# YujiaoShi/HighlyAccurate

Hardware: AMD Instinct MI355X
Metric: image-pairs/sec through N-iter LM pose loop, KITTI shapes (higher is better)
Workload: dtype bf16; 1 GPU; BASELINE configs[1]: LM_S2GP.forward(mode='test'), sat 512x512, grd 256x1024, VGG-16 two-branch, level 3, 5 LM iters x 3 levels, 3-DoF, random-init weights; pairs_per_gpu=32, global_batch=32, parallelism=batch-sharded x1, no collective

## Files before the change

highlyaccurate_amd/csrc/conv_kernels.h:

```cpp
#pragma once
#include "common.h"
#include <type_traits>

typedef __bf16 bf16;
typedef _Float16 f16;
using f32x16 = __attribute__((ext_vector_type(16))) float;
using bf16x8 = __attribute__((ext_vector_type(8))) __bf16;
using f16x8 = __attribute__((ext_vector_type(8))) _Float16;
using f16x4 = __attribute__((ext_vector_type(4))) _Float16;

struct split32 {
  float v;
  split32() = default;
  __host__ __device__ explicit split32(float f) : v(f) {}
  __host__ __device__ explicit operator float() const { return v; }
};
template <typename T> struct Prec { static constexpr bool SPLIT = false; static constexpr int CEPL = 16 / (int)sizeof(T); };
template <> struct Prec<split32> { static constexpr bool SPLIT = true; static constexpr int CEPL = 8; };

__device__ __host__ __forceinline__ float split_scale(unsigned amax_bits) {
  int E = (int)(amax_bits >> 23) & 0xff;
  E = E < 81 ? 81 : (E > 201 ? 201 : E);
  const unsigned bits = (unsigned)(127 + 141 - E) << 23;
  float f;
  __builtin_memcpy(&f, &bits, 4);
  return f;
}
__device__ __forceinline__ void split4(float x0, float x1, float x2, float x3, float s, uint2& hi, uint2& lo) {
  unsigned h01, h23, l01, l23;
  asm("v_fma_mixlo_f16 %0, %4, %8, 0\n\t"
      "v_fma_mixlo_f16 %1, %6, %8, 0\n\t"
      "v_fma_mixhi_f16 %0, %5, %8, 0\n\t"
      "v_fma_mixhi_f16 %1, %7, %8, 0\n\t"
      "v_fma_mixlo_f16 %2, %4, %8, -%0 op_sel_hi:[0,0,1]\n\t"
      "v_fma_mixlo_f16 %3, %6, %8, -%1 op_sel_hi:[0,0,1]\n\t"
      "v_fma_mixhi_f16 %2, %5, %8, -%0 op_sel:[0,0,1] op_sel_hi:[0,0,1]\n\t"
      "v_fma_mixhi_f16 %3, %7, %8, -%1 op_sel:[0,0,1] op_sel_hi:[0,0,1]"
      : "=&v"(h01), "=&v"(h23), "=&v"(l01), "=&v"(l23) : "v"(x0), "v"(x1), "v"(x2), "v"(x3), "v"(s));
  hi = make_uint2(h01, h23);
  lo = make_uint2(l01, l23);
}

#ifndef HLA_TU_DTYPE
#define HLA_TU_DTYPE -1
#endif
#if HLA_TU_DTYPE == 0
typedef float TuT;
#elif HLA_TU_DTYPE == 1
typedef bf16 TuT;
#elif HLA_TU_DTYPE == 2
typedef f16 TuT;
#elif HLA_TU_DTYPE == 3
typedef split32 TuT;
#endif

template <typename T> __device__ __forceinline__ void mma16(f32x16& acc, const uint4& w, const uint4& p);
template <> __device__ __forceinline__ void mma16<bf16>(f32x16& acc, const uint4& w, const uint4& p) {
  acc = __builtin_amdgcn_mfma_f32_32x32x16_bf16(__builtin_bit_cast(bf16x8, w), __builtin_bit_cast(bf16x8, p), acc, 0, 0, 0);
}
template <> __device__ __forceinline__ void mma16<f16>(f32x16& acc, const uint4& w, const uint4& p) {
  acc = __builtin_amdgcn_mfma_f32_32x32x16_f16(__builtin_bit_cast(f16x8, w), __builtin_bit_cast(f16x8, p), acc, 0, 0, 0);
}
template <> __device__ __forceinline__ void mma16<split32>(f32x16& acc, const uint4& w, const uint4& p) {
  acc = __builtin_amdgcn_mfma_f32_32x32x16_f16(__builtin_bit_cast(f16x8, w), __builtin_bit_cast(f16x8, p), acc, 0, 0, 0);
}
template <> __device__ __forceinline__ void mma16<float>(f32x16& acc, const uint4& w, const uint4& p) {
  acc = __builtin_amdgcn_mfma_f32_32x32x2f32(__uint_as_float(w.x), __uint_as_float(p.x), acc, 0, 0, 0);
  acc = __builtin_amdgcn_mfma_f32_32x32x2f32(__uint_as_float(w.y), __uint_as_float(p.y), acc, 0, 0, 0);
  acc = __builtin_amdgcn_mfma_f32_32x32x2f32(__uint_as_float(w.z), __uint_as_float(p.z), acc, 0, 0, 0);
  acc = __builtin_amdgcn_mfma_f32_32x32x2f32(__uint_as_float(w.w), __uint_as_float(p.w), acc, 0, 0, 0);
}

typedef short v4s __attribute__((ext_vector_type(4)));

template <typename T> struct KStep;
template <> struct KStep<bf16> { static constexpr int PX = 16; };
template <> struct KStep<f16> { static constexpr int PX = 16; };
template <> struct KStep<float> { static constexpr int PX = 8; };

template <typename T> __device__ __forceinline__ uint4 frag_kmajor(const char* tile, int stride, int px0, int ch0, int lane);
template <> __device__ __forceinline__ uint4 frag_kmajor<bf16>(const char* tile, int stride, int px0, int ch0, int lane) {
  const int t = lane & 15, i0 = ch0 + 16 * ((lane >> 4) & 1), k0 = px0 + 8 * (lane >> 5);
  const char* p = tile + (k0 + (t >> 2)) * stride + (i0 + 4 * (t & 3)) * 2;
  const v4s lo = __builtin_amdgcn_ds_read_tr16_b64_v4i16((__attribute__((address_space(3))) v4s*)(p));
  const v4s hi = __builtin_amdgcn_ds_read_tr16_b64_v4i16((__attribute__((address_space(3))) v4s*)(p + 4 * stride));
  uint4 r;
  __builtin_memcpy(&r.x, &lo, 8);
  __builtin_memcpy(&r.z, &hi, 8);
  return r;
}
template <> __device__ __forceinline__ uint4 frag_kmajor<f16>(const char* tile, int stride, int px0, int ch0, int lane) {
  return frag_kmajor<bf16>(tile, stride, px0, ch0, lane);
}
template <> __device__ __forceinline__ uint4 frag_kmajor<float>(const char* tile, int stride, int px0, int ch0, int lane) {
  const char* p = tile + (px0 + (lane >> 5)) * stride + (ch0 + (lane & 31)) * 4;
  uint4 r;
  r.x = *(const unsigned*)(p); r.y = *(const unsigned*)(p + 2 * stride);
  r.z = *(const unsigned*)(p + 4 * stride); r.w = *(const unsigned*)(p + 6 * stride);
  return r;
}
template <typename T> __device__ __forceinline__ uint4 frag_ones();
template <> __device__ __forceinline__ uint4 frag_ones<bf16>() { return make_uint4(0x3F803F80u, 0x3F803F80u, 0x3F803F80u, 0x3F803F80u); }
template <> __device__ __forceinline__ uint4 frag_ones<f16>() { return make_uint4(0x3C003C00u, 0x3C003C00u, 0x3C003C00u, 0x3C003C00u); }
template <> __device__ __forceinline__ uint4 frag_ones<float>() { return make_uint4(0x3F800000u, 0x3F800000u, 0x3F800000u, 0x3F800000u); }

__device__ __forceinline__ void store4(bf16* p, float a, float b, float c, float d) {
  const bf16 h[4] = {(bf16)a, (bf16)b, (bf16)c, (bf16)d};
  *(uint2*)p = __builtin_bit_cast(uint2, h);
}
__device__ __forceinline__ void store4(f16* p, float a, float b, float c, float d) {
  const f16 h[4] = {(f16)a, (f16)b, (f16)c, (f16)d};
  *(uint2*)p = __builtin_bit_cast(uint2, h);
}
__device__ __forceinline__ void store4(float* p, float a, float b, float c, float d) {
  *(float4*)p = make_float4(a, b, c, d);
}
__device__ __forceinline__ void store4(split32* p, float a, float b, float c, float d) {
  *(float4*)p = make_float4(a, b, c, d);
}
__device__ __forceinline__ void store4(unsigned char* p, float a, float b, float c, float d) {
  *(unsigned*)p = (unsigned)a | ((unsigned)b << 8) | ((unsigned)c << 16) | ((unsigned)d << 24);
}
__device__ __forceinline__ float to_f32(bf16 v) { return (float)v; }
__device__ __forceinline__ float to_f32(f16 v) { return (float)v; }
__device__ __forceinline__ float to_f32(float v) { return v; }
__device__ __forceinline__ float to_f32(split32 v) { return v.v; }
__device__ __forceinline__ float wave_max_f32(float v) {
#pragma unroll
  for (int o = 32; o > 0; o >>= 1) v = fmaxf(v, __shfl_xor(v, o, 64));
  return v;
}

__device__ __forceinline__ int xcd_contiguous(int bid, int nb) {
  const int q = nb >> 3, r = nb & 7, xcd = bid & 7;
  return (xcd < r ? xcd * (q + 1) : r * (q + 1) + (xcd - r) * q) + (bid >> 3);
}

struct ConvArgs {
  const void* src1;
  const void* src2;
  const uint4* wpk;
  const float* bias;
  void* out_act;
  float* out_raw;
  int raw16;
  double* sumsq;
  int C1, C2, up1;
  int B, H, W, Cout;
  int relu_act;
  int tiles_x, tiles_y;
  int row_begin;
  int src_row_lo;
  int add_row_lo;
  const int* dyn;
  int dyn_desc;
  const unsigned char* unpool_idx;
  const void* mask_act;
  const void* add_src;
  unsigned char* idx_out;
  int pool_sum;
  const unsigned* amax1;
  const unsigned* amax2;
  unsigned* amax_out;
  const float* wscale;
  const float* wg0_x;
  size_t wg0_x_plane;
  float* wg0_part;
#if HLA_CONV_STAMPS
  unsigned long long* stamps;
#endif
};
#if HLA_CONV_STAMPS
#define HLA_STAMP(K) do { if (a.stamps) { const unsigned long long ts_ = __builtin_readcyclecounter(); \
    if ((threadIdx.x & 63) == 0) a.stamps[((size_t)(blockIdx.y * gridDim.x + blockIdx.x) * 4 + (threadIdx.x >> 6)) * HLA_STAMP_N + (K)] = ts_; } } while (0)
#define HLA_STAMP_HWID() do { if (a.stamps && (threadIdx.x & 63) == 0) { \
    const unsigned long long hw_ = __builtin_amdgcn_s_getreg((31 << 11) | (0 << 6) | 4), xc_ = __builtin_amdgcn_s_getreg((31 << 11) | (0 << 6) | 20); \
    a.stamps[((size_t)(blockIdx.y * gridDim.x + blockIdx.x) * 4 + (threadIdx.x >> 6)) * HLA_STAMP_N + 7] = hw_ | (xc_ << 32); } } while (0)
#else
#define HLA_STAMP(K) do {} while (0)
#define HLA_STAMP_HWID() do {} while (0)
#endif

struct ConvDyn {
  int n_live;
  int list;
  int src_bands;
  int add_bands;
};
struct PixBox { int y0, y1, x0, x1; };

constexpr int HWID = 34;
constexpr int SB = 64;
constexpr int PSTR = 64;
__device__ __forceinline__ int halo_key(int hx) { return (hx >> 2) & 3; }
__device__ __forceinline__ int halo_off(int pix, int hx, int slot) { return pix * PSTR + ((slot ^ halo_key(hx)) << 4); }
constexpr int HALO_TAP0 = 2, HALO_TAP1 = 6;
constexpr int HLA_CONV_DMA_TAP = 1;
struct FragOff { int o[3][2]; };
__device__ __forceinline__ FragOff frag_offsets(int lane, int row0) {
  const int x = lane & 31, g = lane >> 5;
  FragOff f;
#pragma unroll
  for (int kx = 0; kx < 3; ++kx)
#pragma unroll
    for (int kg = 0; kg < 2; ++kg) f.o[kx][kg] = halo_off(row0 * HWID + x + kx, x + kx, g | (kg << 1));
  return f;
}

__device__ __forceinline__ float lane_xor1(float v) {
  return __int_as_float(__builtin_amdgcn_update_dpp(0, __float_as_int(v), 0xB1, 0xF, 0xF, false));
}

template <typename E, int NT> struct RowStager {
  static constexpr int CW = NT * 32, PITCH = CW * (int)sizeof(E) + 16, CPP = CW * (int)sizeof(E) / 16;
  static __device__ __forceinline__ void put(char* stage, int px, int ch, float v0, float v1, float v2, float v3) {
    store4((E*)(stage + px * PITCH) + ch, v0, v1, v2, v3);
  }
  template <bool PLAIN = false, int GG = 2>
  static __device__ __forceinline__ float flush(const char* stage, E* dst, int npx, int npx_valid, int Cout, int lane,
                                                const E* mask = nullptr, const E* add = nullptr,
                                                int add_px_lo = 0, int add_px_hi = 1 << 30) {
    float vmax = 0.f;
    const int chunks = npx * CPP;
    constexpr int EPV = 16 / (int)sizeof(E), NIT = 32 * CPP / 64;
    if (PLAIN || !(mask || add)) {
#pragma unroll
      for (int c0 = 0; c0 < 32 * CPP; c0 += 64) {
        const int c = c0 + lane;
        if (c0 < chunks && c < chunks) {
          const int px = c / CPP, part = c % CPP;
          if (px < npx_valid) {
            const unsigned off = (unsigned)px * (unsigned)Cout * (unsigned)sizeof(E) + part * 16;
            *(uint4*)((char*)dst + off) = *(const uint4*)(stage + px * PITCH + part * 16);
          }
        }
      }
      return vmax;
    }
    constexpr int G = NIT < GG ? NIT : GG;
#pragma unroll
    for (int g0 = 0; g0 < NIT; g0 += G) {
      bool ok[G], ap[G];
      unsigned off[G];
      int pxs[G], parts[G];
      uint4 mk[G], ad[G];
#pragma unroll
      for (int k = 0; k < G; ++k) {
        const int c0 = (g0 + k) * 64, c = c0 + lane;
        const int px = c / CPP, part = c % CPP;
        ok[k] = c0 < chunks && c < chunks && px < npx_valid;
        pxs[k] = px; parts[k] = part;
        off[k] = ok[k] ? (unsigned)px * (unsigned)Cout * (unsigned)sizeof(E) + part * 16 : 0u;
        ap[k] = add && ok[k] && px >= add_px_lo && px < add_px_hi;
      }
      if (mask) {
#pragma unroll
        for (int k = 0; k < G; ++k) mk[k] = *(const uint4*)((const char*)mask + off[k]);
      }
      if (add) {
#pragma unroll
        for (int k = 0; k < G; ++k) ad[k] = *(const uint4*)((const char*)add + (ap[k] ? off[k] : 0u));
      }
#pragma unroll
      for (int k = 0; k < G; ++k) {
        if (ok[k]) {
          uint4 v = *(const uint4*)(stage + pxs[k] * PITCH + parts[k] * 16);
          E e[EPV], m[EPV], a2[EPV];
          __builtin_memcpy(e, &v, 16);
          if (mask) __builtin_memcpy(m, &mk[k], 16);
          if (add) __builtin_memcpy(a2, &ad[k], 16);
#pragma unroll
          for (int j = 0; j < EPV; ++j) {
            float f = (float)e[j];
            if (mask && !((float)m[j] > 0.f)) f = 0.f;
            if (ap[k]) f += (float)a2[j];
            e[j] = (E)f;
            vmax = fmaxf(vmax, fabsf(f));
          }
          __builtin_memcpy(&v, e, 16);
          *(uint4*)((char*)dst + off[k]) = v;
        }
      }
    }
    return vmax;
  }
};

enum { EPI_GENERIC = 0,
       EPI_ACT = 1,
       EPI_ACT_RAW = 2,
       EPI_ACT_RAW_NOBIAS = 3,
       EPI_DGRAD = 4,
       EPI_DGRAD_WG0 = 5 };
__host__ __device__ __forceinline__ int epilogue_mode(const ConvArgs& a) {
  if (a.wg0_part) return EPI_DGRAD_WG0;
  if (a.mask_act && a.out_act && !a.relu_act && !a.bias && !a.out_raw && !a.sumsq && !a.idx_out && !a.pool_sum) return EPI_DGRAD;
  if (!a.out_act && a.out_raw && a.raw16 && a.sumsq && !a.bias && !a.mask_act && !a.add_src && !a.idx_out && !a.pool_sum)
    return EPI_ACT_RAW_NOBIAS;
  if (a.mask_act || a.add_src || a.idx_out || a.pool_sum || !a.out_act || !a.relu_act) return EPI_GENERIC;
  if (!a.out_raw) return a.sumsq ? EPI_GENERIC : EPI_ACT;
  return a.sumsq ? (a.bias ? EPI_ACT_RAW : EPI_ACT_RAW_NOBIAS) : EPI_GENERIC;
}
template <typename T, int MT, int NT, bool POOL, int EPI = EPI_GENERIC, bool R16 = false, int STGW = 0>
__device__ __forceinline__ void conv_epilogue(f32x16 (&acc)[MT][NT], const ConvArgs& a, int b, int yrow0, int x0,
                                              int cb, float* red, char* stage, float dsc = 1.f,
                                              PixBox addb = PixBox{0, 1 << 30, 0, 1 << 30},
                                              const float4* prebias = nullptr) {
  using RawT = std::conditional_t<R16, f16, float>;
  constexpr bool GEN = EPI == EPI_GENERIC, RAW = EPI == EPI_ACT_RAW || EPI == EPI_ACT_RAW_NOBIAS, DG = EPI == EPI_DGRAD;
  constexpr bool NOBIAS = EPI == EPI_ACT_RAW_NOBIAS || DG || sizeof(T) == 2;
  const bool has_raw = GEN ? a.out_raw != nullptr : RAW;
  const bool has_act = GEN ? a.out_act != nullptr : true;
  const bool relu = GEN ? a.relu_act != 0 : !DG;
  const bool pool_sum = GEN && a.pool_sum;
  const bool has_sumsq = GEN ? a.sumsq != nullptr : RAW;
  int tid = threadIdx.x;
  asm volatile("" : "+v"(tid));
  const int lane = tid & 63, wv = __builtin_amdgcn_readfirstlane(tid >> 6), x = lane & 31, g = lane >> 5;
  const int Ho = POOL ? a.H >> 1 : a.H, Wo = POOL ? a.W >> 1 : a.W;
  constexpr int NPX = POOL ? 16 : 32;
  float4 bias[NT][4];
#pragma unroll
  for (int j = 0; j < NT; ++j)
#pragma unroll
    for (int q = 0; q < 4; ++q)
      bias[j][q] = make_float4(0.f, 0.f, 0.f, 0.f);
  if (!NOBIAS && prebias) {
#pragma unroll
    for (int j = 0; j < NT; ++j)
#pragma unroll
      for (int q = 0; q < 4; ++q) bias[j][q] = prebias[j * 4 + q];
  } else if (!NOBIAS && a.bias) {
#pragma unroll
    for (int j = 0; j < NT; ++j)
#pragma unroll
      for (int q = 0; q < 4; ++q) bias[j][q] = *(const float4*)(a.bias + cb + j * 32 + q * 8 + g * 4);
  }
  const int xo0 = POOL ? x0 >> 1 : x0;
  const int nvalid = min(NPX, Wo - xo0);
  float ss = 0.f, mx = 0.f;
  constexpr int ROWB = 32 * RowStager<T, NT>::PITCH;
  constexpr bool BATCH = EPI == EPI_ACT && STGW >= 2 * ROWB;
  if constexpr (BATCH) {
    constexpr int STEP = POOL ? 2 : 1, NR = MT / STEP;
    constexpr int RB = STGW / ROWB >= NR ? NR : 2;
    static_assert(NR % RB == 0, "row batches");
#pragma unroll
    for (int r0 = 0; r0 < NR; r0 += RB) {
#pragma unroll
      for (int rr = 0; rr < RB; ++rr) {
        const int i = (r0 + rr) * STEP;
        const bool lane_ok = (yrow0 + i < a.H) && (x0 + x < a.W) && (!POOL || !(x & 1));
        const int px = POOL ? x >> 1 : x;
#pragma unroll
        for (int j = 0; j < NT; ++j)
#pragma unroll
          for (int q = 0; q < 4; ++q) {
            float w[4];
#pragma unroll
            for (int e = 0; e < 4; ++e) {
              float t = acc[i][j][q * 4 + e];
              if (POOL) {
                t = fmaxf(t, acc[i + 1][j][q * 4 + e]);
                t = fmaxf(t, lane_xor1(t));
              }
              if (Prec<T>::SPLIT) t *= dsc;
              w[e] = t;
            }
            if (!NOBIAS) { w[0] += bias[j][q].x; w[1] += bias[j][q].y; w[2] += bias[j][q].z; w[3] += bias[j][q].w; }
            w[0] = fmaxf(w[0], 0.f); w[1] = fmaxf(w[1], 0.f); w[2] = fmaxf(w[2], 0.f); w[3] = fmaxf(w[3], 0.f);
            if (Prec<T>::SPLIT && lane_ok) mx = fmaxf(fmaxf(mx, fmaxf(w[0], w[1])), fmaxf(w[2], w[3]));
            if (!POOL || !(x & 1)) RowStager<T, NT>::put(stage + rr * ROWB, px, j * 32 + q * 8 + g * 4, w[0], w[1], w[2], w[3]);
          }
      }
      __builtin_amdgcn_sched_barrier(0);
#pragma unroll
      for (int rr = 0; rr < RB; ++rr) {
        const int y = yrow0 + (r0 + rr) * STEP;
        const size_t pix0 = ((size_t)b * Ho + (POOL ? y >> 1 : y)) * Wo + xo0;
        if (y < a.H) RowStager<T, NT>::template flush<true>(stage + rr * ROWB, (T*)a.out_act + pix0 * a.Cout + cb, NPX, nvalid, a.Cout, lane);
      }
      __builtin_amdgcn_sched_barrier(0);
    }
  }
#pragma unroll
  for (int i = 0; i < (BATCH ? 0 : MT); i += (POOL ? 2 : 1)) {
    const int y = yrow0 + i;
    const int yo = POOL ? y >> 1 : y;
    const bool row_ok = y < a.H;
    const bool lane_ok = row_ok && (x0 + x < a.W) && (!POOL || !(x & 1));
    const int px = POOL ? x >> 1 : x;
    float v[NT][4][4];
#pragma unroll
    for (int j = 0; j < NT; ++j)
#pragma unroll
      for (int q = 0; q < 4; ++q) {
#pragma unroll
        for (int e = 0; e < 4; ++e) {
          float t = acc[i][j][q * 4 + e];
          if (POOL) {
            const float u = acc[i + 1][j][q * 4 + e];
            if (pool_sum) {
              t += u;
              t += lane_xor1(t);
            } else {
              t = fmaxf(t, u);
              t = fmaxf(t, lane_xor1(t));
            }
          }
          if (Prec<T>::SPLIT) t *= dsc;
          v[j][q][e] = t;
        }
        if (!NOBIAS) { v[j][q][0] += bias[j][q].x; v[j][q][1] += bias[j][q].y; v[j][q][2] += bias[j][q].z; v[j][q][3] += bias[j][q].w; }
      }
    const size_t pix0 = ((size_t)b * Ho + yo) * Wo + xo0;
    constexpr bool ONE_PASS = RAW && sizeof(T) == 2;
    if constexpr (ONE_PASS) {
      char* stage2 = stage + 32 * RowStager<RawT, NT>::PITCH;
      if (!POOL || !(x & 1)) {
#pragma unroll
        for (int j = 0; j < NT; ++j)
#pragma unroll
          for (int q = 0; q < 4; ++q) {
            float w0 = v[j][q][0], w1 = v[j][q][1], w2 = v[j][q][2], w3 = v[j][q][3];
            if (R16) {
              w0 = (float)(f16)fminf(fmaxf(w0, -65504.f), 65504.f); w1 = (float)(f16)fminf(fmaxf(w1, -65504.f), 65504.f);
              w2 = (float)(f16)fminf(fmaxf(w2, -65504.f), 65504.f); w3 = (float)(f16)fminf(fmaxf(w3, -65504.f), 65504.f);
            }
            RowStager<RawT, NT>::put(stage, px, j * 32 + q * 8 + g * 4, w0, w1, w2, w3);
            if (lane_ok) ss += w0 * w0 + w1 * w1 + w2 * w2 + w3 * w3;
            if (a.out_act)
              RowStager<T, NT>::put(stage2, px, j * 32 + q * 8 + g * 4, fmaxf(w0, 0.f), fmaxf(w1, 0.f), fmaxf(w2, 0.f), fmaxf(w3, 0.f));
          }
      }
      asm volatile("" : "+v"(ss));
      __builtin_amdgcn_sched_barrier(0);
      if (row_ok) {
        RowStager<RawT, NT>::template flush<true>(stage, (RawT*)a.out_raw + pix0 * a.Cout + cb, NPX, nvalid, a.Cout, lane);
        if (a.out_act) RowStager<T, NT>::template flush<true>(stage2, (T*)a.out_act + pix0 * a.Cout + cb, NPX, nvalid, a.Cout, lane);
      }
      __builtin_amdgcn_sched_barrier(0);
      continue;
    }
    if (has_raw) {
      if (!POOL || !(x & 1)) {
#pragma unroll
        for (int j = 0; j < NT; ++j)
#pragma unroll
          for (int q = 0; q < 4; ++q) {
            RowStager<float, NT>::put(stage, px, j * 32 + q * 8 + g * 4, v[j][q][0], v[j][q][1], v[j][q][2], v[j][q][3]);
            if (lane_ok) ss += v[j][q][0] * v[j][q][0] + v[j][q][1] * v[j][q][1] + v[j][q][2] * v[j][q][2] + v[j][q][3] * v[j][q][3];
          }
      }
      if (row_ok) RowStager<float, NT>::template flush<true>(stage, a.out_raw + pix0 * a.Cout + cb, NPX, nvalid, a.Cout, lane);
    }
    if (has_act) {
      if (!POOL || !(x & 1)) {
#pragma unroll
        for (int j = 0; j < NT; ++j)
#pragma unroll
          for (int q = 0; q < 4; ++q) {
            float w0 = v[j][q][0], w1 = v[j][q][1], w2 = v[j][q][2], w3 = v[j][q][3];
            if (relu) { w0 = fmaxf(w0, 0.f); w1 = fmaxf(w1, 0.f); w2 = fmaxf(w2, 0.f); w3 = fmaxf(w3, 0.f); }
            if (Prec<T>::SPLIT && lane_ok && !((GEN || DG) && (a.mask_act || a.add_src)))
              mx = fmaxf(fmaxf(mx, fmaxf(fabsf(w0), fabsf(w1))), fmaxf(fabsf(w2), fabsf(w3)));
            RowStager<T, NT>::put(stage, px, j * 32 + q * 8 + g * 4, w0, w1, w2, w3);
          }
      }
      const size_t o = pix0 * a.Cout + cb;
      if (GEN || DG) {
        if (row_ok) {
          const float fm = RowStager<T, NT>::template flush<false, (MT >= 4 ? 4 : 2)>(stage, (T*)a.out_act + o, NPX, nvalid, a.Cout, lane,
                                                   a.mask_act ? (const T*)a.mask_act + o : nullptr,
                                                   (a.add_src && yo >= max(a.add_row_lo, addb.y0) && yo < addb.y1) ? (const T*)a.add_src + o : nullptr,
                                                   addb.x0 - xo0, addb.x1 - xo0);
          if (Prec<T>::SPLIT) mx = fmaxf(mx, fm);
        }
      } else {
        if (row_ok) RowStager<T, NT>::template flush<true>(stage, (T*)a.out_act + o, NPX, nvalid, a.Cout, lane);
      }
    }
    if (GEN && POOL && a.idx_out) {
#pragma unroll
      for (int j = 0; j < NT; ++j)
#pragma unroll
        for (int q = 0; q < 4; ++q) {
          float am[4];
#pragma unroll
          for (int e = 0; e < 4; ++e) {
            const float t0 = acc[i][j][q * 4 + e], u = acc[i + 1][j][q * 4 + e];
            const float rown = u > t0 ? 1.f : 0.f;
            const float t = fmaxf(t0, u);
            const float t2 = lane_xor1(t), r2 = lane_xor1(rown);
            am[e] = t2 > t ? 2.f * r2 + 1.f : 2.f * rown;
          }
          if (!(x & 1)) RowStager<unsigned char, NT>::put(stage, px, j * 32 + q * 8 + g * 4, am[0], am[1], am[2], am[3]);
        }
      if (row_ok) RowStager<unsigned char, NT>::flush(stage, a.idx_out + pix0 * a.Cout + cb, NPX, nvalid, a.Cout, lane);
    }
  }
  const bool want_max = Prec<T>::SPLIT && a.amax_out;
  if (has_sumsq || want_max) {
    ss = wave_sum_f32(ss);
    if (want_max) mx = wave_max_f32(mx);
    if (lane == 0) { red[wv] = ss; red[4 + wv] = mx; }
    __syncthreads();
    if (tid == 0) {
      if (has_sumsq) {
        const int np = a.tiles_x * a.tiles_y * gridDim.y;
        const int tile = (xcd_contiguous(blockIdx.x, gridDim.x) % (a.tiles_x * a.tiles_y)) * gridDim.y + blockIdx.y;
        a.sumsq[(size_t)b * np + tile] = ((double)red[0] + (double)red[1]) + ((double)red[2] + (double)red[3]);
      }
      if (want_max) {
        const unsigned mb = __float_as_uint(fmaxf(fmaxf(red[4], red[5]), fmaxf(red[6], red[7])));
        if (mb > __hip_atomic_load(a.amax_out + b, __ATOMIC_RELAXED, __HIP_MEMORY_SCOPE_AGENT)) atomicMax(a.amax_out + b, mb);
      }
    }
  }
}

template <typename T, int MT>
__device__ __forceinline__ void conv_epilogue_wg0(f32x16 (&acc)[MT][1], const ConvArgs& a, int b, int y0, int x0, char* lds, float dsc) {
  constexpr bool SPLIT = Prec<T>::SPLIT;
  using ET = std::conditional_t<SPLIT, float, T>;
  using FT = std::conditional_t<SPLIT, f16, ET>;
  constexpr int TH = 2 * MT, IH = TH + 2, IW = 48;
  constexpr int PITCH = RowStager<ET, 1>::PITCH, CPP = RowStager<ET, 1>::CPP, NIT = 32 * CPP / 64, EPV = 16 / (int)sizeof(ET);
  constexpr int HP = RowStager<f16, 1>::PITCH, HTILE = 32 * HP;
  constexpr int KPX = KStep<FT>::PX, STG = 5120;
  static_assert(32 * PITCH <= STG && 2 * HTILE <= STG, "wave stager");
  static_assert(4 * STG + 3 * IH * IW * 4 + 2 * 16 * 64 * 4 + 16 <= 2 * (TH + 2) * HWID * PSTR, "fits the halo buffers");
  int tid = threadIdx.x;
  asm volatile("" : "+v"(tid));
  const int lane = tid & 63, wv = __builtin_amdgcn_readfirstlane(tid >> 6), wm = wv >> 1, wn = wv & 1, x = lane & 31, g = lane >> 5;
  char* stage = lds + wv * STG;
  float* in = (float*)(lds + 4 * STG);
  float* xr = in + 3 * IH * IW;
  float* redm = xr + 2 * 16 * 64;
  const int nvalid = min(32, a.W - x0), cb = wn * 32;

  int pxs[NIT], parts[NIT];
  unsigned voff[NIT];
#pragma unroll
  for (int k = 0; k < NIT; ++k) {
    const int c = k * 64 + lane;
    pxs[k] = c / CPP; parts[k] = c % CPP;
    voff[k] = pxs[k] < nvalid ? (unsigned)pxs[k] * 64u * (unsigned)sizeof(ET) + parts[k] * 16 : 0u;
  }
  constexpr int PRE = sizeof(ET) == 2 ? MT : 2;
  uint4 mk[MT][NIT];
  auto load_mask = [&](int i) __attribute__((always_inline)) {
    const int y = min(y0 + wm * MT + i, a.H - 1);
    const char* mrow = (const char*)((const ET*)a.mask_act + (((size_t)b * a.H + y) * a.W + x0) * 64 + cb);
#pragma unroll
    for (int k = 0; k < NIT; ++k) mk[i][k] = *(const uint4*)(mrow + voff[k]);
  };
#pragma unroll
  for (int i = 0; i < PRE; ++i) load_mask(i);

  constexpr int NIN = (3 * IH * IW + 255) / 256;
  float vin[NIN], amx = 0.f;
#pragma unroll
  for (int it = 0; it < NIN; ++it) {
    const int e = tid + it * 256;
    const int c = e / (IH * IW), r = e % (IH * IW), iy = r / IW, ix = r % IW;
    const int y = y0 - 1 + iy, xx = x0 - 1 + ix;
    vin[it] = 0.f;
    if (e < 3 * IH * IW && ix < HWID && y >= 0 && y < a.H && xx >= 0 && xx < a.W)
      vin[it] = a.wg0_x[((size_t)b * 3 + c) * a.wg0_x_plane + (size_t)y * a.W + xx];
  }
#pragma unroll
  for (int it = 0; it < NIN; ++it) {
    const int e = tid + it * 256;
    if (e < 3 * IH * IW) in[e] = vin[it];
    if (SPLIT) amx = fmaxf(amx, fabsf(vin[it]));
  }
  if (SPLIT) {
    amx = wave_max_f32(amx);
    if (lane == 0) redm[wv] = amx;
  }
  __syncthreads();
  float s_in = 1.f;
  if (SPLIT) s_in = split_scale(__float_as_uint(fmaxf(fmaxf(redm[0], redm[1]), fmaxf(redm[2], redm[3]))));

  f32x16 accw;
#pragma unroll
  for (int r = 0; r < 16; ++r) accw[r] = 0.f;
  const int j = lane & 31, g5 = lane >> 5;
  const int jc = j < 27 ? j / 9 : 0, jky = (j % 9) / 3, jkx = j % 3;
#pragma unroll
  for (int i = 0; i < MT; ++i) {
    if (i + PRE < MT) load_mask(i + PRE);
    const int rt = wm * MT + i;
    const bool row_ok = y0 + rt < a.H;
    float sG = 1.f;
    if (SPLIT) {
      float m = 0.f;
#pragma unroll
      for (int r = 0; r < 16; ++r) m = fmaxf(m, fabsf(acc[i][0][r]));
      sG = split_scale(__float_as_uint(wave_max_f32(m) * dsc));
    }
#pragma unroll
    for (int q = 0; q < 4; ++q) {
      float w0 = acc[i][0][q * 4 + 0], w1 = acc[i][0][q * 4 + 1], w2 = acc[i][0][q * 4 + 2], w3 = acc[i][0][q * 4 + 3];
      if (SPLIT) { w0 *= dsc; w1 *= dsc; w2 *= dsc; w3 *= dsc; }
      RowStager<ET, 1>::put(stage, x, q * 8 + g * 4, w0, w1, w2, w3);
    }
    uint4 v[NIT];
#pragma unroll
    for (int k = 0; k < NIT; ++k) {
      v[k] = *(const uint4*)(stage + pxs[k] * PITCH + parts[k] * 16);
      ET e[EPV], m[EPV];
      __builtin_memcpy(e, &v[k], 16);
      __builtin_memcpy(m, &mk[i][k], 16);
      const bool ok = row_ok && pxs[k] < nvalid;
#pragma unroll
      for (int t = 0; t < EPV; ++t)
        if (!ok || !((float)m[t] > 0.f)) e[t] = (ET)0.f;
      __builtin_memcpy(&v[k], e, 16);
    }
    if constexpr (SPLIT) {
#pragma unroll
      for (int k = 0; k < NIT; ++k) {
        uint2 hi, lo;
        split4(__uint_as_float(v[k].x), __uint_as_float(v[k].y), __uint_as_float(v[k].z), __uint_as_float(v[k].w), sG, hi, lo);
        *(uint2*)(stage + pxs[k] * HP + parts[k] * 8) = hi;
        *(uint2*)(stage + HTILE + pxs[k] * HP + parts[k] * 8) = lo;
      }
    } else {
#pragma unroll
      for (int k = 0; k < NIT; ++k) *(uint4*)(stage + pxs[k] * PITCH + parts[k] * 16) = v[k];
    }
    if (row_ok) {
      f32x16 tmp;
      if (SPLIT) {
#pragma unroll
        for (int r = 0; r < 16; ++r) tmp[r] = 0.f;
      }
#pragma unroll
      for (int kk = 0; kk < 32 / KPX; ++kk) {
        const float* row = in + (jc * IH + rt + jky) * IW + jkx + kk * KPX;
        if constexpr (SPLIT) {
          float xs[8];
#pragma unroll
          for (int jj = 0; jj < 8; ++jj) xs[jj] = j < 27 ? row[8 * g5 + jj] : 0.f;
          uint2 h0, l0, h1, l1;
          split4(xs[0], xs[1], xs[2], xs[3], s_in, h0, l0);
          split4(xs[4], xs[5], xs[6], xs[7], s_in, h1, l1);
          uint4 bhi = make_uint4(h0.x, h0.y, h1.x, h1.y);
          const uint4 blo = make_uint4(l0.x, l0.y, l1.x, l1.y);
          if (j == 27) bhi = frag_ones<f16>();
          const uint4 ahi = frag_kmajor<f16>(stage, HP, kk * KPX, 0, lane), alo = frag_kmajor<f16>(stage + HTILE, HP, kk * KPX, 0, lane);
          mma16<f16>(tmp, ahi, bhi);
          mma16<f16>(tmp, alo, bhi);
          mma16<f16>(tmp, ahi, blo);
        } else {
          const uint4 A = frag_kmajor<ET>(stage, PITCH, kk * KPX, 0, lane);
          ET e[EPV];
#pragma unroll
          for (int jj = 0; jj < EPV; ++jj) {
            const int k = sizeof(ET) == 2 ? 8 * g5 + jj : 2 * jj + g5;
            e[jj] = (ET)(j < 27 ? row[k] : (j == 27 ? 1.f : 0.f));
          }
          mma16<ET>(accw, A, __builtin_bit_cast(uint4, e));
        }
      }
      if (SPLIT) {
        const float ds = j == 27 ? 1.f / sG : 1.f / (sG * s_in);
#pragma unroll
        for (int r = 0; r < 16; ++r) accw[r] += tmp[r] * ds;
      }
    }
  }
  if (wm == 1) {
#pragma unroll
    for (int r = 0; r < 16; ++r) xr[(wn * 16 + r) * 64 + lane] = accw[r];
  }
  __syncthreads();
  if (wm == 0) {
    float* dst = a.wg0_part + (size_t)blockIdx.x * 64 * 32;
#pragma unroll
    for (int r = 0; r < 16; ++r) {
      const int co = cb + (r & 3) + 8 * (r >> 2) + 4 * g5;
      dst[co * 32 + j] = accw[r] + xr[(wn * 16 + r) * 64 + lane];
    }
  }
}

template <typename T, int MT, int NT, int WD, int PF = (NT == 1 ? 4 : 3)>
struct WeightRing {
  static constexpr int RS = WD + 1;
  uint4 wb[RS][2][NT];
  static constexpr int PFD = PF;
  uint4 pf[PFD + 1];
  const uint4* wq[NT];

  __device__ __forceinline__ void prime() {
#pragma unroll
    for (int d = 0; d < WD; ++d)
#pragma unroll
      for (int kg = 0; kg < 2; ++kg)
#pragma unroll
        for (int j = 0; j < NT; ++j) wb[d][kg][j] = wq[j][(d * 2 + kg) * 64];
  }
  __device__ __forceinline__ void next_stage() {
#pragma unroll
    for (int j = 0; j < NT; ++j) wq[j] += 18 * 64;
    if (9 % RS != 0) {
      uint4 tmp[WD][2][NT];
#pragma unroll
      for (int d = 0; d < WD; ++d)
#pragma unroll
        for (int kg = 0; kg < 2; ++kg)
#pragma unroll
          for (int j = 0; j < NT; ++j) tmp[d][kg][j] = wb[(9 + d) % RS][kg][j];
#pragma unroll
      for (int d = 0; d < WD; ++d)
#pragma unroll
        for (int kg = 0; kg < 2; ++kg)
#pragma unroll
          for (int j = 0; j < NT; ++j) wb[d][kg][j] = tmp[d][kg][j];
    }
  }
};

__device__ __forceinline__ void stagger_priority() {
  const unsigned slot = __builtin_amdgcn_s_getreg((3 << 11) | (0 << 6) | 4);
  if (slot & 1) __builtin_amdgcn_s_setprio(1);
}

template <typename T, int MT, int NT, int WD, int PF, typename Mid>
__device__ __forceinline__ void stage_mma(f32x16 (&acc)[MT][NT], const char* cur, const FragOff& fo,
                                          WeightRing<T, MT, NT, WD, PF>& ring, Mid&& mid) {
  constexpr int RS = WD + 1;
#pragma unroll
  for (int tap = 0; tap < 9; ++tap) {
#pragma unroll
    for (int kg = 0; kg < 2; ++kg)
#pragma unroll
      for (int j = 0; j < NT; ++j) ring.wb[(tap + WD) % RS][kg][j] = ring.wq[j][((tap + WD) * 2 + kg) * 64];
    mid(tap);
    constexpr int FPT = MT * 2, DEPTH = PF;
    auto frag_ptr = [&](int f) {
      const int tp = tap + f / FPT, r = f % FPT;
      return cur + fo.o[tp % 3][r & 1] + (tp / 3 + (r >> 1)) * HWID * PSTR;
    };
    if (tap == 0) {
#pragma unroll
      for (int f = 0; f < DEPTH; ++f) ring.pf[f] = *(const uint4*)frag_ptr(f);
    }
    __builtin_amdgcn_sched_barrier(0);
#pragma unroll
    for (int f = 0; f < FPT; ++f) {
      const int slot = (tap * FPT + f) % (DEPTH + 1), nslot = (tap * FPT + f + DEPTH) % (DEPTH + 1);
      if (tap * FPT + f + DEPTH < 9 * FPT) ring.pf[nslot] = *(const uint4*)frag_ptr(f + DEPTH);
      const int i = f >> 1, kg = f & 1;
      if constexpr (Prec<T>::SPLIT) {
#pragma unroll
        for (int c = 0; c < (kg == 0 ? 2 : 1); ++c)
#pragma unroll
          for (int j = 0; j < NT; ++j) mma16<T>(acc[i][j], ring.wb[tap % RS][c][j], ring.pf[slot]);
      } else {
#pragma unroll
        for (int j = 0; j < NT; ++j) mma16<T>(acc[i][j], ring.wb[tap % RS][kg][j], ring.pf[slot]);
      }
      __builtin_amdgcn_sched_barrier(0);
    }
  }
  ring.next_stage();
}

template <typename T, int MT, int NT, int WM, int WN, bool POOL, int WD, bool UNPOOL = false>
__global__ __launch_bounds__(256, NT == 1 ? 3 : 2) void conv3x3_kernel(ConvArgs a) {
  static_assert(WM * WN == 4, "4 waves per block");
  constexpr int EPL = 16 / sizeof(T), KC = SB / sizeof(T);
  constexpr int TH = WM * MT, HPIX = (TH + 2) * HWID;
  constexpr int NPIECE = (HPIX * 4 + 255) / 256;
  constexpr bool DMA = sizeof(T) == 2 && !UNPOOL && !Prec<T>::SPLIT;
  constexpr int BUF = (DMA ? NPIECE * 64 : HPIX) * PSTR;
  constexpr int NHALF = (NPIECE + 1) / 2;
  constexpr int STG = 32 * (RowStager<float, NT>::PITCH + (sizeof(T) == 2 ? RowStager<T, NT>::PITCH : 0));
  constexpr int LDSB = 2 * BUF > 4 * STG ? 2 * BUF : 4 * STG;
  __shared__ __attribute__((aligned(16))) char lds[LDSB];
  __shared__ float red[8];

  HLA_STAMP(0);
  HLA_STAMP_HWID();
  const int t = threadIdx.x, lane = t & 63, wv = __builtin_amdgcn_readfirstlane(t >> 6), wm = wv / WN, wn = wv % WN;
  const int sy0 = a.src_row_lo, sy1 = a.H;
  int tx, ty, b;
  struct { int lo0, lo1, lo2, hi0, hi1, hi2; } sb = {0, 0, 0, a.W, a.W, a.W};
  if (a.dyn) {
    const ConvDyn& d = *(const ConvDyn*)(a.dyn + a.dyn_desc);
    const int nl = d.n_live, nlive = nl * a.B;
    if ((int)blockIdx.x >= nlive) return;
    int bid = xcd_contiguous(blockIdx.x, nlive);
    b = bid / nl;
    const int e = a.dyn[d.list + bid % nl];
    ty = e >> 16; tx = e & 0xffff;
    if (d.src_bands >= 0) {
      const int sh = (a.up1 || a.unpool_idx) ? 1 : 0, nb = ((a.H >> sh) + 7) >> 3, yy = a.row_begin + ty * TH;
      const int b0 = min(max(yy - 1, 0) >> sh >> 3, nb - 1), b1 = min(yy >> sh >> 3, nb - 1), b2 = min((yy + TH) >> sh >> 3, nb - 1);
      sb.lo0 = a.dyn[d.src_bands + 2 * b0] << sh; sb.hi0 = min(a.dyn[d.src_bands + 2 * b0 + 1] << sh, a.W);
      sb.lo1 = a.dyn[d.src_bands + 2 * b1] << sh; sb.hi1 = min(a.dyn[d.src_bands + 2 * b1 + 1] << sh, a.W);
      sb.lo2 = a.dyn[d.src_bands + 2 * b2] << sh; sb.hi2 = min(a.dyn[d.src_bands + 2 * b2 + 1] << sh, a.W);
    }
  } else {
    int bid = xcd_contiguous(blockIdx.x, gridDim.x);
    tx = bid % a.tiles_x; bid /= a.tiles_x;
    ty = bid % a.tiles_y;
    b = bid / a.tiles_y;
  }
  const int y0 = a.row_begin + ty * TH, x0 = tx * 32;
  const int nstage = (a.C1 + a.C2) / KC;
  const int part = t & 3, pbase = t >> 2;
  float sx = 1.f, dsc = 1.f;
  if constexpr (Prec<T>::SPLIT) {
    unsigned m = a.amax1[b];
    if (a.amax2) m = max(m, a.amax2[b]);
    sx = split_scale(m);
    dsc = 1.f / (sx * *a.wscale);
  }

  constexpr int ES = (int)sizeof(T);
  const int sh1 = (a.up1 || a.unpool_idx) ? 1 : 0, Hs1 = a.H >> sh1, Ws1 = a.W >> sh1;
  const char* s1b = (const char*)a.src1 + (size_t)b * Hs1 * Ws1 * a.C1 * ES;
  const char* s2b = (const char*)a.src2 + (size_t)b * a.H * a.W * a.C2 * ES;
  const unsigned char* idxb = a.unpool_idx ? a.unpool_idx + (size_t)b * Hs1 * Ws1 * a.C1 : nullptr;
  int off1[NPIECE], off2[NPIECE], wo[NPIECE];
  {
    const int lo0 = __builtin_amdgcn_readfirstlane(sb.lo0), lo1 = __builtin_amdgcn_readfirstlane(sb.lo1),
              lo2 = __builtin_amdgcn_readfirstlane(sb.lo2), hi0 = __builtin_amdgcn_readfirstlane(sb.hi0),
              hi1 = __builtin_amdgcn_readfirstlane(sb.hi1), hi2 = __builtin_amdgcn_readfirstlane(sb.hi2);
#pragma unroll
    for (int i = 0; i < NPIECE; ++i) {
      const int pix = pbase + 64 * i;
      const int hy = pix / HWID, hx = pix - hy * HWID;
      const int y = y0 - 1 + hy, x = x0 - 1 + hx;
      const int xlo = hy == 0 ? lo0 : (hy == TH + 1 ? lo2 : lo1), xhi = hy == 0 ? hi0 : (hy == TH + 1 ? hi2 : hi1);
      const bool ok = pix < HPIX && y >= sy0 && y < sy1 && x >= xlo && x < xhi;
      const int psrc = DMA ? (part ^ halo_key(hx)) : part;
      constexpr int BAD = DMA ? (int)0x80000000 : -1;
      off1[i] = ok ? ((((y >> sh1) * Ws1 + (x >> sh1)) * a.C1 * ES + psrc * 16) | (DMA ? 0 : (((y & 1) << 1) | (x & 1)))) : BAD;
      off2[i] = ok ? ((y * a.W + x) * a.C2 * ES + psrc * 16) : BAD;
      wo[i] = pix >= HPIX ? -1 : (Prec<T>::SPLIT ? halo_off(pix, hx, part >> 1) + (part & 1) * 8 : halo_off(pix, hx, part));
    }
  }
  constexpr int IDW = UNPOOL ? (EPL == 8 ? 2 : 1) : 1;
  struct StageIds { unsigned w[NHALF][IDW]; };
  auto load_stage = [&](int sg, int half, uint4 (&st)[NHALF], StageIds& ids) __attribute__((always_inline)) {
    const int c0 = sg * KC;
    const bool first = c0 < a.C1;
    const char* base = first ? s1b + (size_t)c0 * ES : s2b + (size_t)(c0 - a.C1) * ES;
#pragma unroll
    for (int ii = 0; ii < NHALF; ++ii) {
      const int i = half * NHALF + ii;
      uint4 v = make_uint4(0, 0, 0, 0);
      const int o = i < NPIECE ? (first ? off1[i] : off2[i]) : -1;
      if constexpr (UNPOOL) {
#pragma unroll
        for (int k = 0; k < IDW; ++k) ids.w[ii][k] = 0xffffffffu;
      }
      if (o >= 0) {
        const unsigned ob = (unsigned)o & ~15u;
        v = *(const uint4*)(base + ob);
        if constexpr (UNPOOL) {
          const unsigned char* idp = idxb + ob / ES + c0;
#pragma unroll
          for (int k = 0; k < IDW; ++k) ids.w[ii][k] = ((const unsigned*)idp)[k];
        }
      }
      st[ii] = v;
    }
  };
  auto write_stage = [&](char* buf, int sg, int half, uint4 (&st)[NHALF], const StageIds& ids) __attribute__((always_inline)) {
#pragma unroll
    for (int ii = 0; ii < NHALF; ++ii) {
      const int i = half * NHALF + ii;
      const int w = i < NPIECE ? wo[i] : -1;
      if constexpr (UNPOOL) {
        const bool first = sg * KC < a.C1;
        const unsigned pos = (unsigned)(i < NPIECE ? (first ? off1[i] : off2[i]) : 0) & 3u;
        uint4 v = st[ii];
        if constexpr (sizeof(T) == 2) {
          typedef short s16x2 __attribute__((ext_vector_type(2)));
          const unsigned m0 = ids.w[ii][0] ^ (pos * 0x01010101u), m1 = ids.w[ii][1] ^ (pos * 0x01010101u);
          auto keep = [](unsigned m, unsigned sel) {
            s16x2 w2 = __builtin_bit_cast(s16x2, __builtin_amdgcn_perm(0u, m, sel));
            w2 = (w2 - (short)1) >> 15;
            return __builtin_bit_cast(unsigned, w2);
          };
          v.x &= keep(m0, 0x0c010c00u); v.y &= keep(m0, 0x0c030c02u);
          v.z &= keep(m1, 0x0c010c00u); v.w &= keep(m1, 0x0c030c02u);
        } else {
          T e[EPL];
          __builtin_memcpy(e, &v, 16);
#pragma unroll
          for (int k = 0; k < EPL; ++k) if (((ids.w[ii][0] >> (8 * k)) & 0xffu) != pos) e[k] = (T)0.f;
          __builtin_memcpy(&v, e, 16);
        }
        st[ii] = v;
      }
      if constexpr (Prec<T>::SPLIT) {
        uint2 hi, lo;
        split4(__uint_as_float(st[ii].x), __uint_as_float(st[ii].y), __uint_as_float(st[ii].z), __uint_as_float(st[ii].w), sx, hi, lo);
        if (w >= 0) { *(uint2*)(buf + w) = hi; *(uint2*)(buf + (w ^ 32)) = lo; }
      } else {
        if (w >= 0) *(uint4*)(buf + w) = st[ii];
      }
    }
  };

  typedef int rsrc_t __attribute__((ext_vector_type(4)));
  rsrc_t rs1 = {0, 0, 0, 0x00020000}, rs2 = {0, 0, 0, 0x00020000};
  unsigned lds_wave = 0;
  if constexpr (DMA) {
    const unsigned long long p1 = (unsigned long long)s1b, p2 = (unsigned long long)s2b;
    rs1[0] = __builtin_amdgcn_readfirstlane((int)(unsigned)p1); rs1[1] = __builtin_amdgcn_readfirstlane((int)(unsigned)(p1 >> 32));
    rs1[2] = __builtin_amdgcn_readfirstlane(Hs1 * Ws1 * a.C1 * ES);
    rs2[0] = __builtin_amdgcn_readfirstlane((int)(unsigned)p2); rs2[1] = __builtin_amdgcn_readfirstlane((int)(unsigned)(p2 >> 32));
    rs2[2] = __builtin_amdgcn_readfirstlane(a.src2 ? a.H * a.W * a.C2 * ES : 0);
    lds_wave = __builtin_amdgcn_readfirstlane((unsigned)(unsigned long long)lds) + wv * (16 * PSTR);
  }
  auto dma_stage = [&](int sg, int bufsel) __attribute__((always_inline)) {
    static_assert(!DMA || NPIECE == 6 || NPIECE == 4, "six pieces per thread (8 x 32 tile) or four (4 x 32)");
    const int c0 = sg * KC;
    const bool first = c0 < a.C1;
    const rsrc_t rs = first ? rs1 : rs2;
    const int soff = (first ? c0 : c0 - a.C1) * ES;
    const unsigned dst = lds_wave + bufsel * BUF;
    unsigned keep;
#define HLA_DMA_HEAD(NDST) "s_nop 4\n\ts_mov_b32 %0, m0\n\ts_mov_b32 m0, %" #NDST "\n\ts_nop 0\n\t"
#define HLA_DMA_LD(K, NRS, NSO) "buffer_load_dwordx4 %" #K ", %" #NRS ", %" #NSO " offen lds\n\t"
#define HLA_DMA_STEP "s_add_u32 m0, m0, 0x1000\n\ts_nop 0\n\t"
    if constexpr (NPIECE == 6) {
#define HLA_DMA6(O)                                                                                                                    \
      asm volatile(HLA_DMA_HEAD(9) HLA_DMA_LD(1, 7, 8) HLA_DMA_STEP HLA_DMA_LD(2, 7, 8) HLA_DMA_STEP HLA_DMA_LD(3, 7, 8) HLA_DMA_STEP    \
                   HLA_DMA_LD(4, 7, 8) HLA_DMA_STEP HLA_DMA_LD(5, 7, 8) HLA_DMA_STEP HLA_DMA_LD(6, 7, 8) "s_mov_b32 m0, %0"             \
                   : "=&s"(keep) : "v"(O[0]), "v"(O[1]), "v"(O[2]), "v"(O[3]), "v"(O[4]), "v"(O[5]), "s"(rs), "s"(soff), "s"(dst)      \
                   : "memory", "scc")
      if (first) HLA_DMA6(off1); else HLA_DMA6(off2);
#undef HLA_DMA6
    } else if constexpr (NPIECE == 4) {
#define HLA_DMA4(O)                                                                                                                    \
      asm volatile(HLA_DMA_HEAD(7) HLA_DMA_LD(1, 5, 6) HLA_DMA_STEP HLA_DMA_LD(2, 5, 6) HLA_DMA_STEP HLA_DMA_LD(3, 5, 6) HLA_DMA_STEP    \
                   HLA_DMA_LD(4, 5, 6) "s_mov_b32 m0, %0"                                                                              \
                   : "=&s"(keep) : "v"(O[0]), "v"(O[1]), "v"(O[2]), "v"(O[3]), "s"(rs), "s"(soff), "s"(dst) : "memory", "scc")
      if (first) HLA_DMA4(off1); else HLA_DMA4(off2);
#undef HLA_DMA4
    }
#undef HLA_DMA_HEAD
#undef HLA_DMA_LD
#undef HLA_DMA_STEP
  };

  const int ntg0 = (blockIdx.y * WN + wn) * NT;
  f32x16 acc[MT][NT];
#pragma unroll
  for (int j = 0; j < NT; ++j)
#pragma unroll
    for (int q = 0; q < 4; ++q) {
      float4 b4 = make_float4(0.f, 0.f, 0.f, 0.f);
      if (sizeof(T) == 2 && a.bias) b4 = *(const float4*)(a.bias + (ntg0 + j) * 32 + q * 8 + (lane >> 5) * 4);
#pragma unroll
      for (int i = 0; i < MT; ++i) {
        acc[i][j][q * 4 + 0] = b4.x; acc[i][j][q * 4 + 1] = b4.y; acc[i][j][q * 4 + 2] = b4.z; acc[i][j][q * 4 + 3] = b4.w;
      }
    }

  const FragOff fo = frag_offsets(lane, wm * MT);
  constexpr int PF = NT == 1 ? (UNPOOL && sizeof(T) == 2 ? 3 : 4) : 3;
  WeightRing<T, MT, NT, WD, PF> ring;
#pragma unroll
  for (int j = 0; j < NT; ++j) ring.wq[j] = a.wpk + (size_t)(ntg0 + j) * nstage * 18 * 64 + lane;

  uint4 st[NHALF];
  StageIds ids;
  ring.prime();
  if constexpr (DMA) {
    dma_stage(0, 0);
    asm volatile("s_waitcnt vmcnt(0)" ::: "memory");
  } else {
    uint4 st1[NHALF];
    StageIds ids1;
    load_stage(0, 0, st, ids);
    load_stage(0, 1, st1, ids1);
    write_stage(lds, 0, 0, st, ids);
    write_stage(lds, 0, 1, st1, ids1);
  }
  __syncthreads();
  HLA_STAMP(1);
  stagger_priority();

  for (int sg = 0; sg < nstage; ++sg) {
    const bool more = sg + 1 < nstage;
    char* nxt = lds + ((sg + 1) & 1) * BUF;
    stage_mma<T, MT, NT, WD, PF>(acc, lds + (sg & 1) * BUF, fo, ring, [&](int tap) __attribute__((always_inline)) {
      if constexpr (DMA) {
        if (tap == HLA_CONV_DMA_TAP && more) dma_stage(sg + 1, (sg + 1) & 1);
      } else {
        if (tap == HALO_TAP0 && more) load_stage(sg + 1, 0, st, ids);
        if (tap == HALO_TAP1 && more) { write_stage(nxt, sg + 1, 0, st, ids); load_stage(sg + 1, 1, st, ids); }
      }
    });
    if constexpr (DMA) {
      static_assert(!DMA || HLA_CONV_DMA_TAP <= 8 - WD, "the halo DMA must be issued before the next stage's weight fragments");
      if (more) asm volatile("s_waitcnt vmcnt(%0)" ::"n"(2 * NT * WD) : "memory");
    } else {
      if (more) write_stage(nxt, sg + 1, 1, st, ids);
    }
    if (sg == 0) HLA_STAMP(2);
    __syncthreads();
    if (sg == 0) HLA_STAMP(3);
  }
  HLA_STAMP(4);
  static_assert((LDSB / 4) % 16 == 0, "stager alignment");
  {
    char* stager = lds + wv * (LDSB / 4);
    const int mode = epilogue_mode(a);
    PixBox addb{a.add_row_lo, 1 << 30, 0, 1 << 30};
    if (a.dyn) {
      const ConvDyn& d = *(const ConvDyn*)(a.dyn + a.dyn_desc);
      if (d.add_bands >= 0) {
        const int band = (POOL ? y0 >> 1 : y0) >> 3;
        addb.x0 = a.dyn[d.add_bands + 2 * band];
        addb.x1 = a.dyn[d.add_bands + 2 * band + 1];
      }
    }
    constexpr bool RAW_SPECIAL = POOL || NT == 1;
    constexpr bool T16 = sizeof(T) == 2;
    if constexpr (UNPOOL && NT == 1 && MT == 4 && WN == 2) {
      if (mode == EPI_DGRAD_WG0) {
        conv_epilogue_wg0<T, MT>(acc, a, b, y0, x0, lds, dsc);
        HLA_STAMP(5);
        return;
      }
    }
    if (mode == EPI_ACT) conv_epilogue<T, MT, NT, POOL, EPI_ACT, false, LDSB / 4>(acc, a, b, y0 + wm * MT, x0, ntg0 * 32, red, stager, dsc, addb);
    else if (T16 && RAW_SPECIAL && a.raw16 && mode == EPI_ACT_RAW)
      conv_epilogue<T, MT, NT, POOL, (T16 && RAW_SPECIAL) ? EPI_ACT_RAW : EPI_GENERIC, T16 && RAW_SPECIAL>(acc, a, b, y0 + wm * MT, x0, ntg0 * 32, red, stager, dsc, addb);
    else if (T16 && a.raw16 && mode == EPI_ACT_RAW_NOBIAS)
      conv_epilogue<T, MT, NT, POOL, T16 ? EPI_ACT_RAW_NOBIAS : EPI_GENERIC, T16>(acc, a, b, y0 + wm * MT, x0, ntg0 * 32, red, stager, dsc, addb);
    else if (RAW_SPECIAL && mode == EPI_ACT_RAW) conv_epilogue<T, MT, NT, POOL, RAW_SPECIAL ? EPI_ACT_RAW : EPI_GENERIC>(acc, a, b, y0 + wm * MT, x0, ntg0 * 32, red, stager, dsc, addb);
    else if (mode == EPI_DGRAD)
      conv_epilogue<T, MT, NT, POOL, EPI_DGRAD>(acc, a, b, y0 + wm * MT, x0, ntg0 * 32, red, stager, dsc, addb);
    else if ((RAW_SPECIAL || sizeof(T) == 2) && mode == EPI_ACT_RAW_NOBIAS)
      conv_epilogue<T, MT, NT, POOL, (RAW_SPECIAL || sizeof(T) == 2) ? EPI_ACT_RAW_NOBIAS : EPI_GENERIC>(acc, a, b, y0 + wm * MT, x0, ntg0 * 32, red, stager, dsc, addb);
    else conv_epilogue<T, MT, NT, POOL, EPI_GENERIC>(acc, a, b, y0 + wm * MT, x0, ntg0 * 32, red, stager, dsc, addb);
  }
  HLA_STAMP(5);
}

struct Conv02Args {
  const float* x;
  size_t x_plane;
  const uint4* w0;
  const float* b0;
  const uint4* w2;
  const float* b2;
  void* out_act;
  void* a0_out;
  unsigned char* idx_out;
  void* a2_out;
  int B, H, W, tiles_x, tiles_y;
  int row_begin;
  const float* wtail;
  unsigned* amax_out;
  unsigned* amax_a2_out;
  unsigned* amax_a0_out;
#if HLA_CONV_STAMPS
  unsigned long long* stamps;
#endif
};

template <typename T> constexpr int conv02_rounds() { return sizeof(T) == 4 ? 2 : 1; }
template <typename T> constexpr int conv02_lds_bytes() {
  return (64 * (int)sizeof(T) / SB) / conv02_rounds<T>() * (10 * HWID * PSTR) + 3 * 12 * 36 * 4;
}

template <typename T, int WD>
__global__ __launch_bounds__(256, Prec<T>::SPLIT ? 2 : 3) void conv02_kernel(Conv02Args a0) {
  constexpr bool SPLIT = Prec<T>::SPLIT;
  constexpr bool FOLD = sizeof(T) == 2 && !SPLIT;
  constexpr int EPL = Prec<T>::CEPL, KC = SB / sizeof(T), NSG = 64 / KC, NFRAG = 32 / (2 * EPL), NH = SPLIT ? 2 : 1;
  constexpr int MT = 4, NT = 1, WN = 2, TH = 8, HPIX = (TH + 2) * HWID, BUF = HPIX * PSTR, IW = 36, IH = 12;
  constexpr int ROUNDS = conv02_rounds<T>(), SPR = NSG / ROUNDS, JPR = 2 / ROUNDS;
  extern __shared__ __attribute__((aligned(16))) char smem[];
  char* lds = smem;
  float* in = (float*)(smem + SPR * BUF);
  __shared__ float red[8];
  __shared__ float red2[4];
  float a0mx = 0.f;
#if HLA_CONV_STAMPS
  struct { unsigned long long* stamps; } a = {a0.stamps};
#endif
  HLA_STAMP(0);
  HLA_STAMP_HWID();

  const int t = threadIdx.x, lane = t & 63, wv = __builtin_amdgcn_readfirstlane(t >> 6), wm = wv / WN, wn = wv % WN;
  int bid = blockIdx.x;
  const int tx = bid % a0.tiles_x; bid /= a0.tiles_x;
  const int ty = bid % a0.tiles_y;
  const int b = bid / a0.tiles_y;
  const int y0 = a0.row_begin + ty * TH, x0 = tx * 32;
  const int x = lane & 31, g = lane >> 5;

  WeightRing<T, MT, NT, WD> ring;
  ring.wq[0] = a0.w2 + (size_t)wn * NSG * 18 * 64 + lane;
  ring.prime();

  float amx = 0.f;
  constexpr int NIN = (3 * IH * IW + 255) / 256;
  float vin[NIN];
#pragma unroll
  for (int it = 0; it < NIN; ++it) {
    const int e = t + it * 256;
    const int c = e / (IH * IW), r = e % (IH * IW), iy = r / IW, ix = r % IW;
    const int y = y0 - 2 + iy, xx = x0 - 2 + ix;
    vin[it] = 0.f;
    if (e < 3 * IH * IW && y >= 0 && y < a0.H && xx >= 0 && xx < a0.W)
      vin[it] = a0.x[((size_t)b * 3 + c) * a0.x_plane + (size_t)y * a0.W + xx];
  }
#pragma unroll
  for (int it = 0; it < NIN; ++it) {
    const int e = t + it * 256;
    if (e < 3 * IH * IW) in[e] = vin[it];
    if (SPLIT) amx = fmaxf(amx, fabsf(vin[it]));
  }
  uint4 wf0[JPR][NFRAG][NH];
  auto load_w0 = [&](int j0) __attribute__((always_inline)) {
#pragma unroll
    for (int jj = 0; jj < JPR; ++jj)
#pragma unroll
      for (int f = 0; f < NFRAG; ++f)
#pragma unroll
        for (int h = 0; h < NH; ++h) wf0[jj][f][h] = a0.w0[(((j0 + jj) * NFRAG + f) * NH + h) * 64 + lane];
  };
  load_w0(0);
  if (SPLIT) {
    amx = wave_max_f32(amx);
    if (lane == 0) red[4 + wv] = amx;
  }
  __syncthreads();
  HLA_STAMP(1);

  float4 bias0[JPR][4];
  auto load_b0 = [&](int j0) __attribute__((always_inline)) {
#pragma unroll
    for (int jj = 0; jj < JPR; ++jj)
#pragma unroll
      for (int q = 0; q < 4; ++q) bias0[jj][q] = *(const float4*)(a0.b0 + (j0 + jj) * 32 + q * 8 + g * 4);
  };
  float s_in = 1.f, s_a0 = 1.f, d0 = 1.f, dsc2 = 1.f;
  if constexpr (SPLIT) {
    const float m = fmaxf(fmaxf(red[4], red[5]), fmaxf(red[6], red[7]));
    float bm = fabsf(a0.b0[lane]);
    bm = wave_max_f32(bm);
    s_in = split_scale(__float_as_uint(m));
    s_a0 = split_scale(__float_as_uint(a0.wtail[16] * m + bm));
    d0 = 1.f / (s_in * a0.wtail[0]);
    dsc2 = 1.f / (s_a0 * a0.wtail[1]);
  }
  f32x16 acc[MT][NT];
  float4 bias2[4];
#pragma unroll
  for (int q = 0; q < 4; ++q) bias2[q] = make_float4(0.f, 0.f, 0.f, 0.f);
  const FragOff fo = frag_offsets(lane, wm * MT);
#pragma unroll
  for (int rd = 0; rd < ROUNDS; ++rd) {
  const int j0 = rd * JPR;
  if (rd == 0 && !FOLD) load_b0(0);
  if (rd > 0) __syncthreads();
  for (int m = wv; m * 32 < HPIX; m += 4) {
    const int p = m * 32 + x, pc = p < HPIX ? p : HPIX - 1;
    const int hy = pc / HWID, hx = pc - hy * HWID;
    const float* ib = in + hy * IW + hx;
    const int yy = y0 - 1 + hy, xx = x0 - 1 + hx;
    const bool inside = yy >= 0 && yy < a0.H && xx >= 0 && xx < a0.W;
    f32x16 c0[2];
#pragma unroll
    for (int j = j0; j < j0 + JPR; ++j)
#pragma unroll
      for (int r = 0; r < 16; ++r) c0[j][r] = 0.f;
#pragma unroll
    for (int f = 0; f < NFRAG; ++f) {
      float ev[EPL];
#pragma unroll
      for (int jj = 0; jj < EPL; ++jj) {
        const int kl = f * 2 * EPL + jj, kh = kl + EPL;
        const int ol = kl < 27 ? (kl / 9) * IH * IW + ((kl % 9) / 3) * IW + (kl % 9) % 3 : 0;
        const int oh = kh < 27 ? (kh / 9) * IH * IW + ((kh % 9) / 3) * IW + (kh % 9) % 3 : 0;
        float v = ib[g ? oh : ol];
        if (kh >= 27 && g) v = (FOLD && kh <= 28) ? 1.f : 0.f;
        if (kl >= 27 && !g) v = (FOLD && kl <= 28) ? 1.f : 0.f;
        ev[jj] = v;
      }
      if constexpr (SPLIT) {
        uint2 h0, l0, h1, l1;
        split4(ev[0], ev[1], ev[2], ev[3], s_in, h0, l0);
        split4(ev[4], ev[5], ev[6], ev[7], s_in, h1, l1);
        const uint4 phi = make_uint4(h0.x, h0.y, h1.x, h1.y), plo = make_uint4(l0.x, l0.y, l1.x, l1.y);
#pragma unroll
        for (int j = j0; j < j0 + JPR; ++j) {
          mma16<T>(c0[j], wf0[j - j0][f][0], phi);
          mma16<T>(c0[j], wf0[j - j0][f][NH - 1], phi);
          mma16<T>(c0[j], wf0[j - j0][f][0], plo);
        }
      } else {
        T e[EPL];
#pragma unroll
        for (int jj = 0; jj < EPL; ++jj) e[jj] = (T)ev[jj];
        uint4 pf = __builtin_bit_cast(uint4, e);
        if (FOLD && !inside) pf = make_uint4(0u, 0u, 0u, 0u);
#pragma unroll
        for (int j = j0; j < j0 + JPR; ++j) mma16<T>(c0[j], wf0[j - j0][f][0], pf);
      }
    }
    if (p < HPIX) {
#pragma unroll
      for (int j = j0; j < j0 + JPR; ++j)
#pragma unroll
        for (int q = 0; q < 4; ++q) {
          const int co = j * 32 + q * 8 + g * 4, sl = co / KC - rd * SPR;
          const int byte = (co % KC) * (SPLIT ? 2 : (int)sizeof(T));
          float v0, v1, v2, v3;
          if constexpr (FOLD) {
            v0 = fmaxf(c0[j][q * 4 + 0], 0.f); v1 = fmaxf(c0[j][q * 4 + 1], 0.f);
            v2 = fmaxf(c0[j][q * 4 + 2], 0.f); v3 = fmaxf(c0[j][q * 4 + 3], 0.f);
          } else {
            const float4 bb = bias0[j - j0][q];
            v0 = fmaxf(c0[j][q * 4 + 0] * d0 + bb.x, 0.f); v1 = fmaxf(c0[j][q * 4 + 1] * d0 + bb.y, 0.f);
            v2 = fmaxf(c0[j][q * 4 + 2] * d0 + bb.z, 0.f); v3 = fmaxf(c0[j][q * 4 + 3] * d0 + bb.w, 0.f);
            if (!inside) v0 = v1 = v2 = v3 = 0.f;
          }
          if constexpr (SPLIT) {
            uint2 hi, lo;
            split4(v0, v1, v2, v3, s_a0, hi, lo);
            *(uint2*)(lds + sl * BUF + halo_off(p, hx, byte >> 4) + (byte & 15)) = hi;
            *(uint2*)(lds + sl * BUF + halo_off(p, hx, 2 + (byte >> 4)) + (byte & 15)) = lo;
          } else {
            store4((T*)(lds + sl * BUF + halo_off(p, hx, byte >> 4) + (byte & 15)), v0, v1, v2, v3);
          }
        }
    }
  }
  HLA_STAMP(2);
  __syncthreads();
  HLA_STAMP(3);

  if (rd == 0) {
#pragma unroll
    for (int q = 0; q < 4; ++q) {
      float4 b4 = make_float4(0.f, 0.f, 0.f, 0.f);
      if (sizeof(T) == 2) b4 = *(const float4*)(a0.b2 + wn * 32 + q * 8 + g * 4);
#pragma unroll
      for (int i = 0; i < MT; ++i) {
        acc[i][0][q * 4 + 0] = b4.x; acc[i][0][q * 4 + 1] = b4.y; acc[i][0][q * 4 + 2] = b4.z; acc[i][0][q * 4 + 3] = b4.w;
      }
    }
  }
  if (rd == 0) stagger_priority();
  if (rd + 1 < ROUNDS) { load_w0(j0 + JPR); if (!FOLD) load_b0(j0 + JPR); }
  else if (sizeof(T) == 4) {
#pragma unroll
    for (int q = 0; q < 4; ++q) bias2[q] = *(const float4*)(a0.b2 + wn * 32 + q * 8 + g * 4);
  }
#pragma unroll 1
  for (int sg = 0; sg < SPR; ++sg)
    stage_mma<T, MT, NT, WD>(acc, lds + sg * BUF, fo, ring, [](int) {});
  HLA_STAMP(4);
  if (rd + 1 < ROUNDS) {
#pragma unroll
    for (int jj = 0; jj < JPR; ++jj) {
#pragma unroll
      for (int f = 0; f < NFRAG; ++f)
#pragma unroll
        for (int h = 0; h < NH; ++h) asm volatile("" : "+v"(wf0[jj][f][h].x), "+v"(wf0[jj][f][h].y), "+v"(wf0[jj][f][h].z), "+v"(wf0[jj][f][h].w));
      if (!FOLD) {
#pragma unroll
        for (int q = 0; q < 4; ++q) asm volatile("" : "+v"(bias0[jj][q].x), "+v"(bias0[jj][q].y), "+v"(bias0[jj][q].z), "+v"(bias0[jj][q].w));
      }
    }
  } else if (sizeof(T) == 4) {
#pragma unroll
    for (int q = 0; q < 4; ++q) asm volatile("" : "+v"(bias2[q].x), "+v"(bias2[q].y), "+v"(bias2[q].z), "+v"(bias2[q].w));
  }
  if (rd + 1 == ROUNDS) __builtin_amdgcn_s_waitcnt(0x0F70);
  if (a0.a0_out) {
    constexpr int PPP = 64 * (int)sizeof(T) / 16 / ROUNDS;
    static_assert(TH * 32 * PPP % 256 == 0, "a0 pieces per thread");
    const size_t a0s = (size_t)a0.H * a0.W * 64 * sizeof(T);
    const unsigned long long pb = (unsigned long long)a0.a0_out + (size_t)b * a0s;
    const void* pu = (const void*)(((unsigned long long)__builtin_amdgcn_readfirstlane((int)(unsigned)(pb >> 32)) << 32) |
                                   (unsigned)__builtin_amdgcn_readfirstlane((int)(unsigned)pb));
    const __amdgpu_buffer_rsrc_t ra = __builtin_amdgcn_make_buffer_rsrc((void*)pu, 0, __builtin_amdgcn_readfirstlane((int)a0s), 0x00020000);
    typedef unsigned u32x4 __attribute__((ext_vector_type(4)));
#pragma unroll
    for (int it = 0; it < TH * 32 * PPP / 256; ++it) {
      const int e = t + it * 256;
      const int pxl = e / PPP, piece = e % PPP, sgi = piece / 4, part = piece % 4;
      const int r = pxl / 32, c = pxl % 32, yy = y0 + r, xx = x0 + c;
      const bool ok = yy < a0.H && xx < a0.W;
      const int off = ok ? (yy * a0.W + xx) * 64 * (int)sizeof(T) + (rd * PPP + piece) * 16 : (int)0x80000000;
      const char* sb = lds + sgi * BUF;
      const int hpix = (r + 1) * HWID + c + 1;
      if constexpr (SPLIT) {
        const f16x4 h = __builtin_bit_cast(f16x4, *(const uint2*)(sb + halo_off(hpix, c + 1, part >> 1) + (part & 1) * 8));
        const f16x4 l = __builtin_bit_cast(f16x4, *(const uint2*)(sb + halo_off(hpix, c + 1, 2 + (part >> 1)) + (part & 1) * 8));
        const float is = 1.f / s_a0;
        const float4 o4 = make_float4(((float)h[0] + (float)l[0]) * is, ((float)h[1] + (float)l[1]) * is,
                                      ((float)h[2] + (float)l[2]) * is, ((float)h[3] + (float)l[3]) * is);
        __builtin_amdgcn_raw_buffer_store_b128(__builtin_bit_cast(u32x4, o4), ra, off, 0, 0);
        if (ok) a0mx = fmaxf(fmaxf(a0mx, fmaxf(o4.x, o4.y)), fmaxf(o4.z, o4.w));
      } else {
        __builtin_amdgcn_raw_buffer_store_b128(__builtin_bit_cast(u32x4, *(const uint4*)(sb + halo_off(hpix, c + 1, part))), ra, off, 0, 0);
      }
    }
  }
  }
  if (SPLIT && a0.a0_out && a0.amax_a0_out) {
    a0mx = wave_max_f32(a0mx);
    if (lane == 0) red2[wv] = a0mx;
  }

#if HLA_CONV_STAMPS
  ConvArgs ae{};
#define a ae
#else
  ConvArgs a{};
#endif
  a.bias = a0.b2; a.out_act = a0.out_act; a.B = a0.B; a.H = a0.H; a.W = a0.W; a.Cout = 64; a.relu_act = 1;
  a.tiles_x = a0.tiles_x; a.tiles_y = a0.tiles_y; a.idx_out = a0.idx_out; a.amax_out = a0.amax_out;
  __syncthreads();
  if (SPLIT && a0.a0_out && a0.amax_a0_out && t == 0) {
    const unsigned mb = __float_as_uint(fmaxf(fmaxf(red2[0], red2[1]), fmaxf(red2[2], red2[3])));
    if (mb > __hip_atomic_load(a0.amax_a0_out + b, __ATOMIC_RELAXED, __HIP_MEMORY_SCOPE_AGENT)) atomicMax(a0.amax_a0_out + b, mb);
  }
  const float4* pb2 = sizeof(T) == 4 ? bias2 : nullptr;
  if (a0.a2_out) {
    ConvArgs f = a;
    f.out_act = a0.a2_out; f.idx_out = nullptr; f.amax_out = a0.amax_a2_out;
    conv_epilogue<T, MT, NT, false, EPI_ACT, false, SPR * BUF / 4>(acc, f, b, y0 + wm * MT, x0, wn * 32, red, lds + wv * (SPR * BUF / 4), dsc2, PixBox{0, 1 << 30, 0, 1 << 30}, pb2);
    if (SPLIT) __syncthreads();
  }
  if (a.idx_out) conv_epilogue<T, MT, NT, true, EPI_GENERIC>(acc, a, b, y0 + wm * MT, x0, wn * 32, red, lds + wv * (SPR * BUF / 4), dsc2, PixBox{0, 1 << 30, 0, 1 << 30}, pb2);
  else conv_epilogue<T, MT, NT, true, EPI_ACT, false, SPR * BUF / 4>(acc, a, b, y0 + wm * MT, x0, wn * 32, red, lds + wv * (SPR * BUF / 4), dsc2, PixBox{0, 1 << 30, 0, 1 << 30}, pb2);
#if HLA_CONV_STAMPS
#undef a
  { struct { unsigned long long* stamps; } a = {a0.stamps}; HLA_STAMP(5); }
#endif
}

template <typename T>
__device__ __forceinline__ void pack_weights_body(const float* __restrict__ w, T* __restrict__ out, int Cout, int Cin, int first,
                                                  size_t e0, size_t stride, const float* __restrict__ b0 = nullptr) {
  constexpr int EPL = 16 / sizeof(T), KC = SB / sizeof(T), NFRAG = 32 / (2 * EPL);
  const size_t total = first == 1 ? (size_t)(Cout / 32) * NFRAG * 64 * EPL : (size_t)Cout * Cin * 9;
  for (size_t e = e0; e < total; e += stride) {
    size_t r = e;
    const int j = r % EPL; r /= EPL;
    const int lane = r % 64; r /= 64;
    float v = 0.f;
    if (first == 1) {
      const int f = r % NFRAG; r /= NFRAG;
      const int nt = (int)r;
      const int k = f * 2 * EPL + (lane >> 5) * EPL + j, cout = nt * 32 + (lane & 31);
      if (k < 27) v = w[(size_t)cout * 27 + k];
      else if (b0 && k == 27) v = (float)(T)b0[cout];
      else if (b0 && k == 28) v = b0[cout] - (float)(T)b0[cout];
    } else {
      const int kg = r % 2; r /= 2;
      const int tap = r % 9; r /= 9;
      const int nsg = Cin / KC;
      const int sg = r % nsg; r /= nsg;
      const int nt = (int)r;
      const int cout = nt * 32 + (lane & 31), cin = sg * KC + kg * 2 * EPL + (lane >> 5) * EPL + j;
      v = first == 2 ? w[((size_t)cin * Cout + cout) * 9 + (8 - tap)] : w[((size_t)cout * Cin + cin) * 9 + tap];
    }
    out[e] = (T)v;
  }
}
template <typename T>
__global__ void pack_weights_kernel(const float* __restrict__ w, T* __restrict__ out, int Cout, int Cin, int first) {
  pack_weights_body<T>(w, out, Cout, Cin, first, (size_t)blockIdx.x * blockDim.x + threadIdx.x, (size_t)gridDim.x * blockDim.x);
}
struct PackTable {
  const float* w[16]; size_t off[16];
  int cout[16], cin[16], first[16];
  const float* b0;
};
template <typename T>
__global__ void pack_weights_multi_kernel(PackTable tb, char* __restrict__ packed) {
  const int l = blockIdx.y;
  pack_weights_body<T>(tb.w[l], (T*)(packed + tb.off[l]), tb.cout[l], tb.cin[l], tb.first[l],
                       (size_t)blockIdx.x * blockDim.x + threadIdx.x, (size_t)gridDim.x * blockDim.x, tb.first[l] == 1 ? tb.b0 : nullptr);
}

struct SplitPackTable {
  const float* w[16]; size_t off[16];
  int cout[16], cin[16], first[16], slot[16];
};
static __device__ __forceinline__ void pack_weights_split_body(const float* __restrict__ w, f16* __restrict__ out, int Cout, int Cin, int first,
                                                               const unsigned* __restrict__ wmax_bits, float* __restrict__ scale_out) {
  const float sw = split_scale(*wmax_bits);
  if (blockIdx.x == 0 && threadIdx.x == 0) *scale_out = sw;
  const size_t total = first == 1 ? (size_t)(Cout / 32) * 2 * 2 * 64 * 8 : (size_t)Cout * Cin * 9 * 2;
  for (size_t e = (size_t)blockIdx.x * blockDim.x + threadIdx.x; e < total; e += (size_t)gridDim.x * blockDim.x) {
    size_t r = e;
    const int j = r % 8; r /= 8;
    const int lane = r % 64; r /= 64;
    const int hl = r % 2; r /= 2;
    float v = 0.f;
    if (first == 1) {
      const int f = r % 2; r /= 2;
      const int nt = (int)r;
      const int k = f * 16 + (lane >> 5) * 8 + j, cout = nt * 32 + (lane & 31);
      if (k < 27) v = w[(size_t)cout * 27 + k];
    } else {
      const int tap = r % 9; r /= 9;
      const int nsg = Cin / 16;
      const int sg = r % nsg; r /= nsg;
      const int nt = (int)r;
      const int cout = nt * 32 + (lane & 31), cin = sg * 16 + (lane >> 5) * 8 + j;
      v = first == 2 ? w[((size_t)cin * Cout + cout) * 9 + (8 - tap)] : w[((size_t)cout * Cin + cin) * 9 + tap];
    }
    v *= sw;
    const f16 h = (f16)v;
    out[e] = hl ? (f16)(v - (float)h) : h;
  }
}
static __global__ void pack_weights_split_kernel(const float* __restrict__ w, f16* __restrict__ out, int Cout, int Cin, int first,
                                          const unsigned* __restrict__ wmax_bits, float* __restrict__ scale_out) {
  pack_weights_split_body(w, out, Cout, Cin, first, wmax_bits, scale_out);
}
static __global__ void pack_weights_split_multi_kernel(SplitPackTable tb, char* __restrict__ packed, const unsigned* __restrict__ amax,
                                                       float* __restrict__ scales) {
  const int l = blockIdx.y;
  pack_weights_split_body(tb.w[l], (f16*)(packed + tb.off[l]), tb.cout[l], tb.cin[l], tb.first[l], amax + tb.slot[l], scales + tb.slot[l]);
}
static __global__ void absmax_multi_kernel(SplitPackTable tb, unsigned* __restrict__ amax, unsigned* __restrict__ l1max0) {
  const int l = blockIdx.y;
  const float* w = tb.w[l];
  const size_t n = (size_t)tb.cout[l] * tb.cin[l] * 9;
  float m = 0.f;
  for (size_t e = (size_t)blockIdx.x * blockDim.x + threadIdx.x; e < n; e += (size_t)gridDim.x * blockDim.x) m = fmaxf(m, fabsf(w[e]));
  m = wave_max_f32(m);
  if ((threadIdx.x & 63) == 0) atomicMax(amax + tb.slot[l], __float_as_uint(m));
  if (tb.first[l] == 1 && l1max0 && blockIdx.x == 0)
    for (size_t r0 = threadIdx.x; r0 * 27 < n; r0 += blockDim.x) {
      float sum = 0.f;
      for (int k = 0; k < 27; ++k) sum += fabsf(w[r0 * 27 + k]);
      atomicMax(l1max0, __float_as_uint(sum));
    }
}

static __global__ void absmax_kernel(const float* __restrict__ w, size_t n, int row, unsigned* __restrict__ amax, unsigned* __restrict__ l1max) {
  float m = 0.f;
  for (size_t e = (size_t)blockIdx.x * blockDim.x + threadIdx.x; e < n; e += (size_t)gridDim.x * blockDim.x) m = fmaxf(m, fabsf(w[e]));
  m = wave_max_f32(m);
  if ((threadIdx.x & 63) == 0) atomicMax(amax, __float_as_uint(m));
  if (l1max && blockIdx.x == 0)
    for (size_t r0 = threadIdx.x; r0 * row < n; r0 += blockDim.x) {
      float s = 0.f;
      for (int k = 0; k < row; ++k) s += fabsf(w[r0 * row + k]);
      atomicMax(l1max, __float_as_uint(s));
    }
}

constexpr int CONF_TH = 8, CONF_TW = 32, CONF_HW = CONF_TW + 2, CONF_HPIX = (CONF_TH + 2) * CONF_HW;
constexpr int CONF_NT = (CONF_HPIX + 31) / 32;
template <typename T, int C>
__global__ __launch_bounds__(256) void conf_kernel(const T* __restrict__ act, const float* __restrict__ w,
                                                   float* __restrict__ out, int B, int H, int W) {
  constexpr int EPL = 16 / sizeof(T), KS = 2 * EPL, NS = C / KS;
  constexpr bool SPLITW = sizeof(T) == 2;
  __shared__ float td[CONF_NT * 32 * 9];
  const int lane = threadIdx.x & 63, wv = threadIdx.x >> 6, n = lane & 31, g = lane >> 5;
  const int tiles_x = (W + CONF_TW - 1) / CONF_TW, tiles_y = (H + CONF_TH - 1) / CONF_TH;
  int bid = blockIdx.x;
  const int x0 = (bid % tiles_x) * CONF_TW; bid /= tiles_x;
  const int y0 = (bid % tiles_y) * CONF_TH;
  const size_t b = bid / tiles_y;
  uint4 wh[NS], wl[SPLITW ? NS : 1];
#pragma unroll
  for (int s = 0; s < NS; ++s) {
    T hi[EPL], lo[EPL];
#pragma unroll
    for (int k = 0; k < EPL; ++k) {
      const float v = n < 9 ? w[(s * KS + g * EPL + k) * 9 + n] : 0.f;
      hi[k] = (T)v;
      lo[k] = (T)(v - to_f32(hi[k]));
    }
    __builtin_memcpy(&wh[s], hi, 16);
    if (SPLITW) __builtin_memcpy(&wl[s], lo, 16);
  }
  for (int t = wv; t < CONF_NT; t += 4) {
    const int hp = t * 32 + n, hy = hp / CONF_HW, hx = hp - hy * CONF_HW, y = y0 - 1 + hy, x = x0 - 1 + hx;
    const bool ok = hp < CONF_HPIX && y >= 0 && y < H && x >= 0 && x < W;
    const T* src = act + ((b * H + (ok ? y : 0)) * W + (ok ? x : 0)) * C + g * EPL;
    uint4 a[NS];
#pragma unroll
    for (int s = 0; s < NS; ++s) a[s] = ok ? *(const uint4*)(src + s * KS) : make_uint4(0, 0, 0, 0);
    f32x16 acc;
#pragma unroll
    for (int r = 0; r < 16; ++r) acc[r] = 0.f;
#pragma unroll
    for (int s = 0; s < NS; ++s) {
      mma16<T>(acc, wh[s], a[s]);
      if (SPLITW) mma16<T>(acc, wl[s], a[s]);
    }
#pragma unroll
    for (int r = 0; r < 8; ++r) {
      const int tap = (r & 3) + 8 * (r >> 2) + 4 * g;
      if (tap < 9) td[hp * 9 + tap] = acc[r];
    }
  }
  __syncthreads();
  const int py = threadIdx.x / CONF_TW, px = threadIdx.x % CONF_TW, y = y0 + py, x = x0 + px;
  if (y < H && x < W) {
    float s = 0.f;
#pragma unroll
    for (int tap = 0; tap < 9; ++tap) s += td[((py + tap / 3) * CONF_HW + px + tap % 3) * 9 + tap];
    const float sg = 1.f / (1.f + __expf(-s));
    out[(b * H + y) * W + x] = 1.f / (1.f + __expf(sg));
  }
}

static __global__ __launch_bounds__(256) void inv_norm_kernel(const double* __restrict__ sumsq, int np, double* __restrict__ inv) {
  __shared__ double sh[4];
  const int b = blockIdx.x;
  double s = 0.0;
  for (int i = threadIdx.x; i < np; i += 256) s += sumsq[(size_t)b * np + i];
  s = wave_sum_f64(s);
  if ((threadIdx.x & 63) == 0) sh[threadIdx.x >> 6] = s;
  __syncthreads();
  if (threadIdx.x == 0) inv[b] = 1.0 / fmax(sqrt((sh[0] + sh[1]) + (sh[2] + sh[3])), 1e-12);
}
struct InvNormArgs { const double* ss[4]; int np[4]; double* inv; int B; };
static __global__ __launch_bounds__(256) void inv_norm_multi_kernel(InvNormArgs a) {
  __shared__ double sh[4];
  const int b = blockIdx.x, l = blockIdx.y, np = a.np[l];
  const double* sumsq = a.ss[l];
  double s = 0.0;
  for (int i = threadIdx.x; i < np; i += 256) s += sumsq[(size_t)b * np + i];
  s = wave_sum_f64(s);
  if ((threadIdx.x & 63) == 0) sh[threadIdx.x >> 6] = s;
  __syncthreads();
  if (threadIdx.x == 0) a.inv[(size_t)l * a.B + b] = 1.0 / fmax(sqrt((sh[0] + sh[1]) + (sh[2] + sh[3])), 1e-12);
}
static __global__ __launch_bounds__(256) void scale_kernel(float* __restrict__ x, const double* __restrict__ inv, size_t per_sample,
                                                    int blocks_per_sample) {
  const int b = blockIdx.x / blocks_per_sample, k = blockIdx.x % blocks_per_sample;
  const double scale = inv[b];
  float4* p = (float4*)(x + (size_t)b * per_sample);
  const size_t n4 = per_sample / 4;
  for (size_t i = (size_t)k * 256 + threadIdx.x; i < n4; i += (size_t)blocks_per_sample * 256) {
    float4 v = p[i];
    v.x = (float)((double)v.x * scale); v.y = (float)((double)v.y * scale);
    v.z = (float)((double)v.z * scale); v.w = (float)((double)v.w * scale);
    p[i] = v;
  }
}


constexpr int CONV_SMALL_GRID = 320;
template <typename T, bool BWD = false>
static bool launch_conv(hipStream_t st, ConvArgs a, bool pool) {
  if (a.unpool_idx && !(BWD && !pool)) {
    hla_set_error("launch_conv: an un-pooled source needs the UNPOOL kernel (backward, no pooling epilogue)");
    return false;
  }
  a.tiles_x = (a.W + 31) / 32;
  a.tiles_y = (a.H - a.row_begin + 7) / 8;
#if HLA_CONV_STAMPS
  a.stamps = nullptr;
  if (g_hla_stamp.buf && g_hla_stamp.counter++ == g_hla_stamp.want) {
    a.stamps = g_hla_stamp.buf;
    g_hla_stamp.grid_x = a.tiles_x * a.tiles_y * a.B; g_hla_stamp.grid_y = a.Cout >= 128 ? a.Cout / 128 : 1;
  }
#endif
  const bool big = a.Cout >= 128;
  const dim3 grid(a.tiles_x * a.tiles_y * a.B, big ? a.Cout / 128 : 1);
  const size_t es = sizeof(T), P = (size_t)a.B * (a.H - a.row_begin) * a.W, Po = pool ? P / 4 : P;
  const double flops = 2.0 * 9.0 * (a.C1 + a.C2) * a.Cout * (double)P + (a.wg0_part ? 2.0 * 27 * 64 * (double)P : 0.0);
  const double bytes = (double)P * ((a.up1 ? a.C1 / 4.0 : a.C1) + a.C2) * es + (double)Po * a.Cout * ((a.out_act ? es : 0) + (a.out_raw ? 4 : 0));
  hla_prof_begin_dyn(a.Cout >= 128 ? (pool ? K_CONV_NT2_POOL : K_CONV_NT2) : (pool ? K_CONV_NT1_POOL : K_CONV_NT1), flops, bytes, st,
                     a.dyn ? a.dyn + a.dyn_desc : nullptr, a.tiles_x * a.tiles_y);
  if constexpr (!BWD) {
    const int gy = big ? a.Cout / 128 : 1;
    if (!a.dyn && !a.sumsq && !a.unpool_idx && a.tiles_x * a.tiles_y * a.B * gy < CONV_SMALL_GRID) {
      a.tiles_y = (a.H - a.row_begin + 3) / 4;
      const dim3 g4(a.tiles_x * a.tiles_y * a.B, gy);
      if (big) {
        if (pool) hipLaunchKernelGGL((conv3x3_kernel<T, 2, 2, 2, 2, true, 1>), g4, dim3(256), 0, st, a);
        else hipLaunchKernelGGL((conv3x3_kernel<T, 2, 2, 2, 2, false, 1>), g4, dim3(256), 0, st, a);
      } else {
        if (pool) hipLaunchKernelGGL((conv3x3_kernel<T, 2, 1, 2, 2, true, 2>), g4, dim3(256), 0, st, a);
        else hipLaunchKernelGGL((conv3x3_kernel<T, 2, 1, 2, 2, false, 2>), g4, dim3(256), 0, st, a);
      }
      hla_prof_end(st);
      return true;
    }
  }
  if (big) {
    if (pool) hipLaunchKernelGGL((conv3x3_kernel<T, 4, 2, 2, 2, true, 1>), grid, dim3(256), 0, st, a);
    else if (BWD && a.unpool_idx) hipLaunchKernelGGL((conv3x3_kernel<T, 4, 2, 2, 2, false, 1, BWD>), grid, dim3(256), 0, st, a);
    else hipLaunchKernelGGL((conv3x3_kernel<T, 4, 2, 2, 2, false, 1>), grid, dim3(256), 0, st, a);
  } else {
    if (pool) hipLaunchKernelGGL((conv3x3_kernel<T, 4, 1, 2, 2, true, 2>), grid, dim3(256), 0, st, a);
    else if (BWD && a.unpool_idx) hipLaunchKernelGGL((conv3x3_kernel<T, 4, 1, 2, 2, false, 2, BWD>), grid, dim3(256), 0, st, a);
    else hipLaunchKernelGGL((conv3x3_kernel<T, 4, 1, 2, 2, false, 2>), grid, dim3(256), 0, st, a);
  }
  hla_prof_end(st);
  return true;
}
```

highlyaccurate_amd/csrc/vgg.hip:

```cpp
#include "conv_kernels.h"
#include "vgg_layers.h"
#include <type_traits>

template <typename T>
void vgg_pack_all(const hla_vgg_params* prm, char* packed, int dtype, hipStream_t st) {
  float* tail = (float*)(packed + packed_offset(kAllLayers, dtype));
  unsigned* scratch = (unsigned*)tail + 32;
  if (Prec<T>::SPLIT) (void)hipMemsetAsync(tail, 0, kPackTailBytes, st);
  if constexpr (!Prec<T>::SPLIT) {
    PackTable tb{};
    tb.b0 = prm->b[0];
    int n = 0;
    for (int l = 0; l < kAllLayers; ++l) {
      if (l >= kPackedLayers && !prm->w[l]) continue;
      tb.w[n] = prm->w[l]; tb.off[n] = packed_offset(l, dtype); tb.cout[n] = kLayers[l].cout; tb.cin[n] = kLayers[l].cin;
      tb.first[n] = l == 0 ? 1 : 0;
      ++n;
    }
    hla_prof_begin(K_PACK, 0, (double)packed_offset(kAllLayers, dtype) * (1.0 + 4.0 / sizeof(T)), st);
    hipLaunchKernelGGL((pack_weights_multi_kernel<T>), dim3(256, n), dim3(256), 0, st, tb, packed);
    hla_prof_end(st);
    return;
  }
  if constexpr (Prec<T>::SPLIT) {
    SplitPackTable tb{};
    int n = 0;
    for (int l = 0; l < kAllLayers; ++l) {
      if (l >= kPackedLayers && !prm->w[l]) continue;
      tb.w[n] = prm->w[l]; tb.off[n] = packed_offset(l, dtype); tb.cout[n] = kLayers[l].cout; tb.cin[n] = kLayers[l].cin;
      tb.first[n] = l == 0 ? 1 : 0; tb.slot[n] = l;
      ++n;
    }
    hla_prof_begin(K_PACK, 0, (double)packed_offset(kAllLayers, dtype) * 3.0, st);
    hipLaunchKernelGGL(absmax_multi_kernel, dim3(64, n), dim3(256), 0, st, tb, scratch, (unsigned*)tail + 16);
    hipLaunchKernelGGL(pack_weights_split_multi_kernel, dim3(256, n), dim3(256), 0, st, tb, packed, (const unsigned*)scratch, tail);
    hla_prof_end(st);
  }
}

template <typename T>
int vgg_forward_t(const float* x, size_t x_plane, const hla_vgg_params* prm, const char* packed, int dtype, void* const feat[4],
                         float* const conf[4], double* inv_norm, char* ws, const VggPlan& pl, int B, int H, int W,
                         int flags, int first_row8, hipStream_t st) {
  const bool level4 = pl.x2r != 0;
  const int NL = level4 ? 4 : 3;
  const bool fold = (flags & HLA_VGG_FOLD_DECODER) != 0;
  auto dH = [&](int d) { return fold ? 2 * (H / d) : H / d; };
  auto dW = [&](int d) { return fold ? (W / d) / 2 : W / d; };
  auto W_ = [&](int l) { return (const uint4*)(packed + packed_offset(l, dtype)); };
  char* w = ws;
  constexpr bool SPLIT = Prec<T>::SPLIT;
  const float* wtail = (const float*)(packed + packed_offset(kAllLayers, dtype));
  unsigned* amax = (unsigned*)(w + pl.amax);
  auto AM = [&](int slot) { return (SPLIT && slot >= 0) ? amax + (size_t)slot * B : (unsigned*)nullptr; };
  if (SPLIT) HLA_CHECK_HIP(hipMemsetAsync(amax, 0, (size_t)kAmaxSlots * B * sizeof(unsigned), st));
  auto conv02 = [&]() -> int {
    Conv02Args a{};
    a.x_plane = x_plane ? x_plane : (size_t)H * W;
    a.x = x; a.w0 = W_(0); a.b0 = prm->b[0]; a.w2 = W_(1); a.b2 = prm->b[1];
    a.out_act = w + pl.x3;
    if (flags & HLA_VGG_SAVE_FOR_BACKWARD) {
      a.a0_out = w + pl.a0;
      a.idx_out = (unsigned char*)(w + pl.idx3);
    }
    if (level4) a.a2_out = w + pl.x2r;
    a.wtail = wtail; a.amax_out = AM(AM_X3); a.amax_a2_out = level4 ? AM(AM_X2) : nullptr;
    a.amax_a0_out = (flags & HLA_VGG_SAVE_FOR_BACKWARD) ? AM(AM_A0) : nullptr;
    const int f0 = (level4 || (flags & HLA_VGG_SAVE_FOR_BACKWARD)) ? 0 : first_row8;
    a.row_begin = f0 ? 8 * f0 - 32 : 0;
    a.B = B; a.H = H; a.W = W; a.tiles_x = (W + 31) / 32; a.tiles_y = (H - a.row_begin + 7) / 8;
    const double P = (double)B * (H - a.row_begin) * W;
    constexpr int lds_bytes = conv02_lds_bytes<T>();
    static HlaPerDeviceOnce attr_once;
    HLA_CHECK_HIP(attr_once.run([] {
      return hipFuncSetAttribute((const void*)conv02_kernel<T, 2>, hipFuncAttributeMaxDynamicSharedMemorySize, lds_bytes);
    }));
#if HLA_CONV_STAMPS
    a.stamps = nullptr;
    if (g_hla_stamp.buf && g_hla_stamp.want <= -10 && g_hla_stamp.want++ == -10) {
      a.stamps = g_hla_stamp.buf; g_hla_stamp.want = -1000;
      g_hla_stamp.grid_x = a.tiles_x * a.tiles_y * B; g_hla_stamp.grid_y = 1;
    }
#endif
    hla_prof_begin(K_CONV02, 2.0 * 9 * (3 + 64) * 64 * P, P * (3 * 4 + 16 * sizeof(T)), st);
    hipLaunchKernelGGL((conv02_kernel<T, 2>), dim3(a.tiles_x * a.tiles_y * B), dim3(256), lds_bytes, st, a);
    hla_prof_end(st);
    return HLA_OK;
  };
  const bool train = flags & HLA_VGG_SAVE_FOR_BACKWARD;
  int np_used[4] = {pl.np[0], pl.np[1], pl.np[2], pl.np[3]};
  bool launch_ok = true;
  auto conv = [&](int l, const void* s1, int C1, int H_, int W_h, void* act, int relu, bool pool, const void* s2 = nullptr,
                  int C2 = 0, int up1 = 0, void* raw = nullptr, double* ss = nullptr, unsigned char* idx = nullptr,
                  int row_begin = 0, int norm_level = -1) {
    ConvArgs a{};
    a.raw16 = (raw && (flags & HLA_VGG_FEAT16)) ? 1 : 0;
    a.row_begin = row_begin < 0 ? 0 : row_begin;
    a.idx_out = train ? idx : nullptr;
    a.src1 = s1; a.src2 = s2;
    a.C1 = C1; a.C2 = C2; a.up1 = up1; a.wpk = W_(l);
    a.bias = kLayers[l].has_bias ? prm->b[l] : nullptr;
    a.out_act = act; a.out_raw = (float*)raw; a.sumsq = ss;
    a.B = B; a.H = H_; a.W = W_h; a.Cout = kLayers[l].cout;
    a.relu_act = relu;
    if (SPLIT) {
      static const signed char kAm[13][3] = {{-1, -1, -1}, {-1, -1, -1}, {AM_X3, -1, AM_A5}, {AM_A5, -1, AM_X8}, {AM_X8, -1, AM_A10},
                                             {AM_A10, -1, AM_A12}, {AM_A12, -1, AM_X15}, {AM_X15, AM_X8, AM_D1A}, {AM_D1A, -1, AM_X18},
                                             {AM_X18, AM_X3, AM_D2A}, {AM_D2A, -1, AM_X21}, {AM_X21, AM_X2, AM_D3A}, {AM_D3A, -1, AM_X24}};
      a.amax1 = AM(kAm[l][0]); a.amax2 = AM(kAm[l][1]); a.amax_out = AM(kAm[l][2]); a.wscale = wtail + l;
    }
    if (!launch_conv<T>(st, a, pool)) launch_ok = false;
    if (norm_level >= 0)
      np_used[norm_level] = ((W_h + 31) / 32) * ((H_ - a.row_begin + 7) / 8) * (a.Cout >= 128 ? a.Cout / 128 : 1);
  };
  const int f = (level4 || train) ? 0 : first_row8;
  const int wc = ((flags & HLA_VGG_WANT_CONF) && conf) ? 1 : 0;
  const int r_c5 = f ? 4 * f - 15 : 0, r_c7 = f ? 4 * f - 14 : 0, r_c10 = f ? 2 * f - 6 : 0, r_c12 = f ? 2 * f - 5 : 0,
            r_c14 = f ? 2 * f - 4 : 0, r_d11 = f ? 2 * f - 2 - wc : 0, r_d13 = f ? 2 * f - 1 - wc : 0,
            r_d21 = f ? 4 * f - 1 - wc : 0, r_d23 = f ? 4 * f - wc : 0;
  if (const int rc = conv02()) return rc;
  conv(2, w + pl.x3, 64, H / 2, W / 2, w + pl.a5, 1, false, nullptr, 0, 0, nullptr, nullptr, nullptr, r_c5);
  conv(3, w + pl.a5, 128, H / 2, W / 2, w + pl.x8, 1, true, nullptr, 0, 0, nullptr, nullptr,
       (unsigned char*)(w + pl.idx8), r_c7);
  conv(4, w + pl.x8, 128, H / 4, W / 4, w + pl.a10, 1, false, nullptr, 0, 0, nullptr, nullptr, nullptr, r_c10);
  conv(5, w + pl.a10, 256, H / 4, W / 4, w + pl.a12, 1, false, nullptr, 0, 0, nullptr, nullptr, nullptr, r_c12);
  conv(6, w + pl.a12, 256, H / 4, W / 4, w + pl.x15r, 1, true, nullptr, 0, 0, feat[0],
       (double*)(w + pl.ss[0]), (unsigned char*)(w + pl.idx15), r_c14, 0);
  conv(7, w + pl.x15r, 256, dH(4), dW(4), w + pl.d1a, 1, false, w + pl.x8, 128, 1, nullptr, nullptr, nullptr, r_d11);
  conv(8, w + pl.d1a, 128, dH(4), dW(4), w + pl.x18r, 1, false, nullptr, 0, 0, feat[1],
       (double*)(w + pl.ss[1]), nullptr, r_d13, 1);
  const bool x21r_dead = !level4 && !wc && !train && (flags & HLA_VGG_FEAT16) && sizeof(T) == 2;
  conv(9, w + pl.x18r, 128, dH(2), dW(2), w + pl.d2a, 1, false, w + pl.x3, 64, 1, nullptr, nullptr, nullptr, r_d21);
  conv(10, w + pl.d2a, 64, dH(2), dW(2), x21r_dead ? (char*)nullptr : w + pl.x21r, 1, false, nullptr, 0, 0, feat[2],
       (double*)(w + pl.ss[2]), nullptr, r_d23, 2);
  if (level4) {
    conv(11, w + pl.x21r, 64, dH(1), dW(1), w + pl.d3a, 1, false, w + pl.x2r, 64, 1);
    conv(12, w + pl.d3a, 64, dH(1), dW(1), w + pl.x24r, 1, false, nullptr, 0, 0, feat[3],
         (double*)(w + pl.ss[3]), nullptr, 0, 3);
  }
  if ((flags & HLA_VGG_WANT_CONF) && conf) {
    using CT = std::conditional_t<SPLIT, float, T>;
    const CT* acts[4] = {(const CT*)(w + pl.x15r), (const CT*)(w + pl.x18r), (const CT*)(w + pl.x21r), (const CT*)(w + pl.x24r)};
    const int Cs[4] = {256, 128, 64, 64}, hs[4] = {H / 8, dH(4), dH(2), dH(1)}, wsz[4] = {W / 8, dW(4), dW(2), dW(1)};
    for (int l = 0; l < NL; ++l) {
      if (!conf[l]) continue;
      const size_t npix = (size_t)B * hs[l] * wsz[l];
      const int grid = B * ((hs[l] + CONF_TH - 1) / CONF_TH) * ((wsz[l] + CONF_TW - 1) / CONF_TW);
      hla_prof_begin(K_CONF, 2.0 * 9 * Cs[l] * (double)npix, (double)npix * (Cs[l] * sizeof(CT) + 4), st);
      if (Cs[l] == 256) hipLaunchKernelGGL((conf_kernel<CT, 256>), dim3(grid), dim3(256), 0, st, acts[l], prm->w[13 + l], conf[l], B, hs[l], wsz[l]);
      else if (Cs[l] == 128) hipLaunchKernelGGL((conf_kernel<CT, 128>), dim3(grid), dim3(256), 0, st, acts[l], prm->w[13 + l], conf[l], B, hs[l], wsz[l]);
      else hipLaunchKernelGGL((conf_kernel<CT, 64>), dim3(grid), dim3(256), 0, st, acts[l], prm->w[13 + l], conf[l], B, hs[l], wsz[l]);
      hla_prof_end(st);
    }
  }
  {
    const size_t per[4] = {(size_t)(H / 8) * (W / 8) * 256, (size_t)(H / 4) * (W / 4) * 128, (size_t)(H / 2) * (W / 2) * 64,
                           (size_t)H * W * 64};
    double* inv = inv_norm ? inv_norm : (double*)(w + pl.inv);
    {
      InvNormArgs ia{};
      double bytes = 0;
      for (int l = 0; l < NL; ++l) { ia.ss[l] = (const double*)(w + pl.ss[l]); ia.np[l] = np_used[l]; bytes += (double)B * pl.np[l] * 8; }
      ia.inv = inv; ia.B = B;
      hla_prof_begin(K_L2NORM, 0, bytes, st);
      hipLaunchKernelGGL(inv_norm_multi_kernel, dim3(B, NL), dim3(256), 0, st, ia);
      hla_prof_end(st);
    }
    for (int l = 0; l < NL; ++l) {
      if (flags & HLA_VGG_DEFER_NORM) continue;
      int bps = (int)(per[l] / 4 / 256 / 4);
      bps = bps < 1 ? 1 : (bps > 64 ? 64 : bps);
      hla_prof_begin(K_L2NORM, 0, (double)B * per[l] * 8, st);
      hipLaunchKernelGGL(scale_kernel, dim3(B * bps), dim3(256), 0, st, (float*)feat[l], inv + (size_t)l * B, per[l], bps);
      hla_prof_end(st);
    }
  }
  HLA_CHECK_HIP(hipGetLastError());
  return launch_ok ? HLA_OK : HLA_ERR_ARG;
}

#if HLA_TU_DTYPE >= 0
template void vgg_pack_all<TuT>(const hla_vgg_params* prm, char* packed, int dtype, hipStream_t st);
template int vgg_forward_t<TuT>(const float* x, size_t x_plane, const hla_vgg_params* prm, const char* packed, int dtype, void* const feat[4],
                              float* const conf[4], double* inv_norm, char* ws, const VggPlan& pl, int B, int H, int W,
                              int flags, int first_row8, hipStream_t st);
#else
#define HLA_EXTERN_T(T) \
  extern template void vgg_pack_all<T>(const hla_vgg_params* prm, char* packed, int dtype, hipStream_t st); \
  extern template int vgg_forward_t<T>(const float* x, size_t x_plane, const hla_vgg_params* prm, const char* packed, int dtype, void* const feat[4],                               float* const conf[4], double* inv_norm, char* ws, const VggPlan& pl, int B, int H, int W,                               int flags, int first_row8, hipStream_t st);
HLA_EXTERN_T(float) HLA_EXTERN_T(bf16) HLA_EXTERN_T(f16) HLA_EXTERN_T(split32)

extern "C" size_t hla_vgg_packed_weight_bytes(int dtype) {
  return packed_offset(kAllLayers, dtype) + (dtype == HLA_F16X3 ? kPackTailBytes : 0);
}

extern "C" int hla_vgg_pack_weights(const hla_vgg_params* params, void* packed, int dtype, hla_stream_t stream) {
  HLA_REQUIRE(params && packed, "hla_vgg_pack_weights: null argument");
  HLA_REQUIRE(hla_dtype_ok(dtype), "hla_vgg_pack_weights: bad dtype %d", dtype);
  HLA_REQUIRE(params->w[0] && params->b[0], "hla_vgg_pack_weights: conv0's weight and bias are required (the bias is packed with it)");
  if (dtype == HLA_BF16) vgg_pack_all<bf16>(params, (char*)packed, dtype, (hipStream_t)stream);
  else if (dtype == HLA_F16) vgg_pack_all<f16>(params, (char*)packed, dtype, (hipStream_t)stream);
  else if (dtype == HLA_F16X3) vgg_pack_all<split32>(params, (char*)packed, dtype, (hipStream_t)stream);
  else vgg_pack_all<float>(params, (char*)packed, dtype, (hipStream_t)stream);
  HLA_CHECK_HIP(hipGetLastError());
  return HLA_OK;
}

extern "C" size_t hla_vgg_workspace_bytes(int B, int H, int W, int level, int dtype) {
  VggPlan p;
  vgg_plan(B, H, W, dtype, true, &p, level == 4);
  return p.total;
}

extern "C" size_t hla_vgg_workspace_bytes_flags(int B, int H, int W, int level, int dtype, int flags) {
  VggPlan p;
  vgg_plan(B, H, W, dtype, true, &p, level == 4, (flags & HLA_VGG_FOLD_DECODER) != 0);
  return p.total;
}

extern "C" int hla_vgg_forward(const float* x, size_t x_plane, const hla_vgg_params* params, const void* packed_weights,
                               void* const feat[4], float* const conf[4], double* inv_norm, void* workspace,
                               size_t workspace_bytes, int B, int H, int W, int level, int dtype, int flags,
                               int first_row8, hla_stream_t stream) {
  HLA_REQUIRE(x && params && packed_weights && feat && workspace, "hla_vgg_forward: null argument");
  HLA_REQUIRE(hla_dtype_ok(dtype), "hla_vgg_forward: dtype must be HLA_F32, HLA_BF16, HLA_F16 or HLA_F16X3 (got %d)", dtype);
  HLA_REQUIRE(B > 0 && H >= 8 && W >= 8 && H % 8 == 0 && W % 8 == 0, "hla_vgg_forward: H and W must be multiples of 8");
  HLA_REQUIRE(x_plane == 0 || x_plane >= (size_t)H * W, "hla_vgg_forward: x_plane (%zu) must be 0 or >= H*W", x_plane);
  HLA_REQUIRE((size_t)H * W * 64 * 4 < ((size_t)1 << 31), "hla_vgg_forward: image too large (H*W must be below 2^23 pixels)");
  HLA_REQUIRE(level == 3 || level == 4, "hla_vgg_forward: level must be 3 (x15,x18,x21) or 4 (+x24), got %d", level);
  HLA_REQUIRE(feat[0] && feat[1] && feat[2], "hla_vgg_forward: feat[0..2] are required");
  HLA_REQUIRE(level == 3 || (feat[3] && params->w[11] && params->w[12]),
              "hla_vgg_forward: level 4 needs feat[3] ([B,H,W,64], 16 real channels) and the zero-padded conv_dec3 weights in w[11], w[12]");
  HLA_REQUIRE(level == 3 || !(flags & HLA_VGG_WANT_CONF) || !conf || !conf[3] || params->w[16], "hla_vgg_forward: conf[3] needs w[16]");
  HLA_REQUIRE(!(flags & HLA_VGG_DEFER_NORM) || inv_norm, "hla_vgg_forward: HLA_VGG_DEFER_NORM needs inv_norm");
  HLA_REQUIRE(!(flags & HLA_VGG_FEAT16) || ((dtype == HLA_BF16 || dtype == HLA_F16) && (flags & HLA_VGG_DEFER_NORM) &&
                                            !(flags & HLA_VGG_SAVE_FOR_BACKWARD) && level == 3),
              "hla_vgg_forward: HLA_VGG_FEAT16 needs dtype HLA_BF16 / HLA_F16, HLA_VGG_DEFER_NORM, level 3 and no HLA_VGG_SAVE_FOR_BACKWARD");
  HLA_REQUIRE(first_row8 == 0 || (first_row8 >= 4 && first_row8 < H / 8), "hla_vgg_forward: first_row8 must be 0 or in [4, H/8)");
  HLA_REQUIRE(!(flags & HLA_VGG_FOLD_DECODER) || (W % 16 == 0 && first_row8 == 0 && !(flags & HLA_VGG_FEAT16)),
              "hla_vgg_forward: HLA_VGG_FOLD_DECODER needs W %% 16 == 0 (folded maps are W/16, W/8, W/4 wide), first_row8 == 0 and no "
              "HLA_VGG_FEAT16 (got W = %d, first_row8 = %d)", W, first_row8);
  VggPlan pl;
  vgg_plan(B, H, W, dtype, (flags & HLA_VGG_SAVE_FOR_BACKWARD) != 0, &pl, level == 4, (flags & HLA_VGG_FOLD_DECODER) != 0);
  if (workspace_bytes < pl.total) {
    hla_set_error("hla_vgg_forward: workspace %zu < %zu", workspace_bytes, pl.total);
    return HLA_ERR_WORKSPACE;
  }
  if (dtype == HLA_BF16)
    return vgg_forward_t<bf16>(x, x_plane, params, (const char*)packed_weights, dtype, feat, conf, inv_norm, (char*)workspace, pl,
                               B, H, W, flags, first_row8, (hipStream_t)stream);
  if (dtype == HLA_F16)
    return vgg_forward_t<f16>(x, x_plane, params, (const char*)packed_weights, dtype, feat, conf, inv_norm, (char*)workspace, pl,
                              B, H, W, flags, first_row8, (hipStream_t)stream);
  if (dtype == HLA_F16X3)
    return vgg_forward_t<split32>(x, x_plane, params, (const char*)packed_weights, dtype, feat, conf, inv_norm, (char*)workspace, pl,
                                  B, H, W, flags, first_row8, (hipStream_t)stream);
  return vgg_forward_t<float>(x, x_plane, params, (const char*)packed_weights, dtype, feat, conf, inv_norm, (char*)workspace, pl,
                              B, H, W, flags, first_row8, (hipStream_t)stream);
}
#endif
```

highlyaccurate_amd/csrc/vgg_layers.h:

```cpp
#pragma once
#include "common.h"

struct LayerDef { int cin, cout, has_bias; };
static const LayerDef kLayers[13] = {
    {3, 64, 1}, {64, 64, 1}, {64, 128, 1}, {128, 128, 1}, {128, 256, 1}, {256, 256, 1}, {256, 256, 1},
    {384, 128, 0}, {128, 128, 0}, {192, 64, 0}, {64, 64, 0},
    {128, 64, 0}, {64, 64, 0}};
constexpr int kPackedLayers = 11;
constexpr int kAllLayers = 13;

static inline size_t hla_elem_bytes(int dtype) { return (dtype == HLA_F32 || dtype == HLA_F16X3) ? 4 : 2; }
constexpr size_t kPackTailBytes = 256;

static inline size_t packed_bytes(int l, int dtype) {
  const size_t es = hla_elem_bytes(dtype);
  if (l == 0) return (size_t)2 * 32 * 32 * es;
  return (size_t)kLayers[l].cin * kLayers[l].cout * 9 * es + 4096;
}
static inline size_t packed_offset(int l, int dtype) {
  size_t o = 0;
  for (int i = 0; i < l; ++i) o += hla_align_up(packed_bytes(i, dtype), 256);
  return o;
}

enum { AM_X3 = 0, AM_A5, AM_X8, AM_A10, AM_A12, AM_X15, AM_D1A, AM_X18, AM_D2A, AM_X21, AM_X2, AM_D3A, AM_X24, AM_A0, kAmaxSlots = 16 };

struct VggPlan {
  size_t x3, a5, x8, a10, a12, x15r, d1a, x18r, d2a, x21r;
  size_t x2r, d3a, x24r;
  size_t ss[4], inv;
  size_t a0, idx3, idx8, idx15;
  size_t amax;
  int np[4];
  size_t total;
};

static inline void vgg_plan(int B, int H, int W, int dtype, bool train, VggPlan* p, bool level4 = false, bool fold = false) {
  const size_t es = hla_elem_bytes(dtype);
  size_t o = 0;
  auto take = [&](size_t bytes) { size_t r = o; o += hla_align_up(bytes, 256); return r; };
  const size_t P = (size_t)B * H * W;
  p->x3 = take(P / 4 * 64 * es);
  p->a5 = take(P / 4 * 128 * es);
  p->x8 = take(P / 16 * 128 * es);
  p->a10 = take(P / 16 * 256 * es);
  p->a12 = take(P / 16 * 256 * es);
  p->x15r = take(P / 64 * 256 * es);
  p->d1a = take(P / 16 * 128 * es);
  p->x18r = take(P / 16 * 128 * es);
  p->d2a = take(P / 4 * 64 * es);
  p->x21r = take(P / 4 * 64 * es);
  auto tiles = [](int h, int w) { return ((h + 7) / 8) * ((w + 31) / 32); };
  auto tiles_f = [&](int h, int w) { return fold ? tiles(2 * h, w / 2) : tiles(h, w); };
  p->np[0] = tiles(H / 4, W / 4) * 2;
  p->np[1] = tiles_f(H / 4, W / 4) * 1;
  p->np[2] = tiles_f(H / 2, W / 2) * 1;
  p->np[3] = tiles_f(H, W) * 1;
  for (int i = 0; i < 4; ++i) p->ss[i] = take((size_t)B * p->np[i] * sizeof(double));
  p->inv = take((size_t)4 * B * sizeof(double));
  p->amax = take((size_t)kAmaxSlots * B * sizeof(unsigned));
  p->x2r = p->d3a = p->x24r = 0;
  if (level4) {
    p->x2r = take(P * 64 * es);
    p->d3a = take(P * 64 * es);
    p->x24r = take(P * 64 * es);
  }
  p->a0 = p->idx3 = p->idx8 = p->idx15 = 0;
  if (train) {
    p->a0 = take(P * 64 * es);
    p->idx3 = take(P / 4 * 64);
    p->idx8 = take(P / 16 * 128);
    p->idx15 = take(P / 64 * 256);
  }
  p->total = o;
}
```

Before: 4998 pairs/s.

## Use 16x16x32 MFMA shape for forward bf16 convolutions with Cout>=128

Adds a 16x16x32 MFMA accumulator layout (four f32x4 tiles per 32x32 block) and routes forward 16-bit conv kernels with Cout>=128 through it. The weight packing, fragment offsets, bias init and epilogue pixel/channel mapping are generalized per shape, and the layer table gains a pool flag so the packer can pick the matching layout. The aim is to use the higher-throughput or better-scheduled smaller MFMA instruction on the large conv layers. The risk is different register pressure, LDS access patterns and epilogue cost, plus layout mismatches between packed weights and kernels.

```diff
diff --git a/highlyaccurate_amd/csrc/conv_kernels.h b/highlyaccurate_amd/csrc/conv_kernels.h
--- a/highlyaccurate_amd/csrc/conv_kernels.h
+++ b/highlyaccurate_amd/csrc/conv_kernels.h
@@ -69,6 +69,32 @@
   acc = __builtin_amdgcn_mfma_f32_32x32x2f32(__uint_as_float(w.y), __uint_as_float(p.y), acc, 0, 0, 0);
   acc = __builtin_amdgcn_mfma_f32_32x32x2f32(__uint_as_float(w.z), __uint_as_float(p.z), acc, 0, 0, 0);
   acc = __builtin_amdgcn_mfma_f32_32x32x2f32(__uint_as_float(w.w), __uint_as_float(p.w), acc, 0, 0, 0);
+}
+
+enum { SHAPE_32x32x16 = 0, SHAPE_16x16x32 = 1 };
+using f32x4 = __attribute__((ext_vector_type(4))) float;
+struct Acc16x16 { f32x4 t[4]; };
+template <int SHAPE> struct AccMap;
+template <> struct AccMap<SHAPE_32x32x16> {
+  using Tile = f32x16;
+  static __device__ __forceinline__ float get(const Tile& a, int q, int e) { return a[q * 4 + e]; }
+  static __device__ __forceinline__ void set(Tile& a, int q, int e, float v) { a[q * 4 + e] = v; }
+  static __device__ __forceinline__ int px(int lane, int) { return lane & 31; }
+  static __device__ __forceinline__ int ch(int lane, int q) { return 8 * q + 4 * (lane >> 5); }
+};
+template <> struct AccMap<SHAPE_16x16x32> {
+  using Tile = Acc16x16;
+  static __device__ __forceinline__ float get(const Tile& a, int q, int e) { return a.t[q][e]; }
+  static __device__ __forceinline__ void set(Tile& a, int q, int e, float v) { a.t[q][e] = v; }
+  static __device__ __forceinline__ int px(int lane, int q) { return 16 * (q >> 1) + (lane & 15); }
+  static __device__ __forceinline__ int ch(int lane, int q) { return 16 * (q & 1) + 4 * (lane >> 4); }
+};
+template <typename T> __device__ __forceinline__ void mma32(f32x4& acc, const uint4& w, const uint4& p);
+template <> __device__ __forceinline__ void mma32<bf16>(f32x4& acc, const uint4& w, const uint4& p) {
+  acc = __builtin_amdgcn_mfma_f32_16x16x32_bf16(__builtin_bit_cast(bf16x8, w), __builtin_bit_cast(bf16x8, p), acc, 0, 0, 0);
+}
+template <> __device__ __forceinline__ void mma32<f16>(f32x4& acc, const uint4& w, const uint4& p) {
+  acc = __builtin_amdgcn_mfma_f32_16x16x32_f16(__builtin_bit_cast(f16x8, w), __builtin_bit_cast(f16x8, p), acc, 0, 0, 0);
 }
 
 typedef short v4s __attribute__((ext_vector_type(4)));
@@ -197,13 +223,22 @@
 constexpr int HALO_TAP0 = 2, HALO_TAP1 = 6;
 constexpr int HLA_CONV_DMA_TAP = 1;
 struct FragOff { int o[3][2]; };
+template <int SHAPE = SHAPE_32x32x16>
 __device__ __forceinline__ FragOff frag_offsets(int lane, int row0) {
-  const int x = lane & 31, g = lane >> 5;
   FragOff f;
-#pragma unroll
-  for (int kx = 0; kx < 3; ++kx)
-#pragma unroll
-    for (int kg = 0; kg < 2; ++kg) f.o[kx][kg] = halo_off(row0 * HWID + x + kx, x + kx, g | (kg << 1));
+  if constexpr (SHAPE == SHAPE_16x16x32) {
+    const int x = lane & 15, slot = lane >> 4;
+#pragma unroll
+    for (int kx = 0; kx < 3; ++kx)
+#pragma unroll
+      for (int p = 0; p < 2; ++p) f.o[kx][p] = halo_off(row0 * HWID + 16 * p + x + kx, 16 * p + x + kx, slot);
+  } else {
+    const int x = lane & 31, g = lane >> 5;
+#pragma unroll
+    for (int kx = 0; kx < 3; ++kx)
+#pragma unroll
+      for (int kg = 0; kg < 2; ++kg) f.o[kx][kg] = halo_off(row0 * HWID + x + kx, x + kx, g | (kg << 1));
+  }
   return f;
 }
 
@@ -301,8 +336,8 @@
   if (!a.out_raw) return a.sumsq ? EPI_GENERIC : EPI_ACT;
   return a.sumsq ? (a.bias ? EPI_ACT_RAW : EPI_ACT_RAW_NOBIAS) : EPI_GENERIC;
 }
-template <typename T, int MT, int NT, bool POOL, int EPI = EPI_GENERIC, bool R16 = false, int STGW = 0>
-__device__ __forceinline__ void conv_epilogue(f32x16 (&acc)[MT][NT], const ConvArgs& a, int b, int yrow0, int x0,
+template <typename T, int MT, int NT, bool POOL, int EPI = EPI_GENERIC, bool R16 = false, int STGW = 0, int SHAPE = SHAPE_32x32x16>
+__device__ __forceinline__ void conv_epilogue(typename AccMap<SHAPE>::Tile (&acc)[MT][NT], const ConvArgs& a, int b, int yrow0, int x0,
                                               int cb, float* red, char* stage, float dsc = 1.f,
                                               PixBox addb = PixBox{0, 1 << 30, 0, 1 << 30},
                                               const float4* prebias = nullptr) {
@@ -316,9 +351,18 @@
   const bool has_sumsq = GEN ? a.sumsq != nullptr : RAW;
   int tid = threadIdx.x;
   asm volatile("" : "+v"(tid));
-  const int lane = tid & 63, wv = __builtin_amdgcn_readfirstlane(tid >> 6), x = lane & 31, g = lane >> 5;
+  const int lane = tid & 63, wv = __builtin_amdgcn_readfirstlane(tid >> 6), even = !POOL || !(lane & 1);
+  using M = AccMap<SHAPE>;
   const int Ho = POOL ? a.H >> 1 : a.H, Wo = POOL ? a.W >> 1 : a.W;
   constexpr int NPX = POOL ? 16 : 32;
+  int pxq[4];
+  bool colok[4];
+#pragma unroll
+  for (int q = 0; q < 4; ++q) {
+    const int xq = M::px(lane, q);
+    pxq[q] = POOL ? xq >> 1 : xq;
+    colok[q] = (x0 + xq < a.W) && even;
+  }
   float4 bias[NT][4];
 #pragma unroll
   for (int j = 0; j < NT; ++j)
@@ -334,7 +378,7 @@
 #pragma unroll
     for (int j = 0; j < NT; ++j)
 #pragma unroll
-      for (int q = 0; q < 4; ++q) bias[j][q] = *(const float4*)(a.bias + cb + j * 32 + q * 8 + g * 4);
+      for (int q = 0; q < 4; ++q) bias[j][q] = *(const float4*)(a.bias + cb + j * 32 + M::ch(lane, q));
   }
   const int xo0 = POOL ? x0 >> 1 : x0;
   const int nvalid = min(NPX, Wo - xo0);
@@ -350,8 +394,7 @@
 #pragma unroll
       for (int rr = 0; rr < RB; ++rr) {
         const int i = (r0 + rr) * STEP;
-        const bool lane_ok = (yrow0 + i < a.H) && (x0 + x < a.W) && (!POOL || !(x & 1));
-        const int px = POOL ? x >> 1 : x;
+        const bool rowok = yrow0 + i < a.H;
 #pragma unroll
         for (int j = 0; j < NT; ++j)
 #pragma unroll
@@ -359,9 +402,9 @@
             float w[4];
 #pragma unroll
             for (int e = 0; e < 4; ++e) {
-              float t = acc[i][j][q * 4 + e];
+              float t = M::get(acc[i][j], q, e);
               if (POOL) {
-                t = fmaxf(t, acc[i + 1][j][q * 4 + e]);
+                t = fmaxf(t, M::get(acc[i + 1][j], q, e));
                 t = fmaxf(t, lane_xor1(t));
               }
               if (Prec<T>::SPLIT) t *= dsc;
@@ -369,8 +412,8 @@
             }
             if (!NOBIAS) { w[0] += bias[j][q].x; w[1] += bias[j][q].y; w[2] += bias[j][q].z; w[3] += bias[j][q].w; }
             w[0] = fmaxf(w[0], 0.f); w[1] = fmaxf(w[1], 0.f); w[2] = fmaxf(w[2], 0.f); w[3] = fmaxf(w[3], 0.f);
-            if (Prec<T>::SPLIT && lane_ok) mx = fmaxf(fmaxf(mx, fmaxf(w[0], w[1])), fmaxf(w[2], w[3]));
-            if (!POOL || !(x & 1)) RowStager<T, NT>::put(stage + rr * ROWB, px, j * 32 + q * 8 + g * 4, w[0], w[1], w[2], w[3]);
+            if (Prec<T>::SPLIT && rowok && colok[q]) mx = fmaxf(fmaxf(mx, fmaxf(w[0], w[1])), fmaxf(w[2], w[3]));
+            if (even) RowStager<T, NT>::put(stage + rr * ROWB, pxq[q], j * 32 + M::ch(lane, q), w[0], w[1], w[2], w[3]);
           }
       }
       __builtin_amdgcn_sched_barrier(0);
@@ -388,8 +431,12 @@
     const int y = yrow0 + i;
     const int yo = POOL ? y >> 1 : y;
     const bool row_ok = y < a.H;
-    const bool lane_ok = row_ok && (x0 + x < a.W) && (!POOL || !(x & 1));
-    const int px = POOL ? x >> 1 : x;
+    const bool lane_ok = row_ok && (x0 + M::px(lane, 0) < a.W) && even;
+    auto quad_ok = [&](int q) { return SHAPE == SHAPE_32x32x16 ? lane_ok : (row_ok && colok[q]); };
+    auto sumsq4 = [&](float s, float v0, float v1, float v2, float v3) {
+      if constexpr (SHAPE == SHAPE_32x32x16) return s + (v0 * v0 + v1 * v1 + v2 * v2 + v3 * v3);
+      else return __builtin_fmaf(v3, v3, __builtin_fmaf(v2, v2, __builtin_fmaf(v1, v1, __builtin_fmaf(v0, v0, s))));
+    };
     float v[NT][4][4];
 #pragma unroll
     for (int j = 0; j < NT; ++j)
@@ -397,9 +444,9 @@
       for (int q = 0; q < 4; ++q) {
 #pragma unroll
         for (int e = 0; e < 4; ++e) {
-          float t = acc[i][j][q * 4 + e];
+          float t = M::get(acc[i][j], q, e);
           if (POOL) {
-            const float u = acc[i + 1][j][q * 4 + e];
+            const float u = M::get(acc[i + 1][j], q, e);
             if (pool_sum) {
               t += u;
               t += lane_xor1(t);
@@ -417,7 +464,7 @@
     constexpr bool ONE_PASS = RAW && sizeof(T) == 2;
     if constexpr (ONE_PASS) {
       char* stage2 = stage + 32 * RowStager<RawT, NT>::PITCH;
-      if (!POOL || !(x & 1)) {
+      if (even) {
 #pragma unroll
         for (int j = 0; j < NT; ++j)
 #pragma unroll
@@ -427,10 +474,10 @@
               w0 = (float)(f16)fminf(fmaxf(w0, -65504.f), 65504.f); w1 = (float)(f16)fminf(fmaxf(w1, -65504.f), 65504.f);
               w2 = (float)(f16)fminf(fmaxf(w2, -65504.f), 65504.f); w3 = (float)(f16)fminf(fmaxf(w3, -65504.f), 65504.f);
             }
-            RowStager<RawT, NT>::put(stage, px, j * 32 + q * 8 + g * 4, w0, w1, w2, w3);
-            if (lane_ok) ss += w0 * w0 + w1 * w1 + w2 * w2 + w3 * w3;
+            RowStager<RawT, NT>::put(stage, pxq[q], j * 32 + M::ch(lane, q), w0, w1, w2, w3);
+            if (quad_ok(q)) ss = sumsq4(ss, w0, w1, w2, w3);
             if (a.out_act)
-              RowStager<T, NT>::put(stage2, px, j * 32 + q * 8 + g * 4, fmaxf(w0, 0.f), fmaxf(w1, 0.f), fmaxf(w2, 0.f), fmaxf(w3, 0.f));
+              RowStager<T, NT>::put(stage2, pxq[q], j * 32 + M::ch(lane, q), fmaxf(w0, 0.f), fmaxf(w1, 0.f), fmaxf(w2, 0.f), fmaxf(w3, 0.f));
           }
       }
       asm volatile("" : "+v"(ss));
@@ -443,28 +490,28 @@
       continue;
     }
     if (has_raw) {
-      if (!POOL || !(x & 1)) {
+      if (even) {
 #pragma unroll
         for (int j = 0; j < NT; ++j)
 #pragma unroll
           for (int q = 0; q < 4; ++q) {
-            RowStager<float, NT>::put(stage, px, j * 32 + q * 8 + g * 4, v[j][q][0], v[j][q][1], v[j][q][2], v[j][q][3]);
-            if (lane_ok) ss += v[j][q][0] * v[j][q][0] + v[j][q][1] * v[j][q][1] + v[j][q][2] * v[j][q][2] + v[j][q][3] * v[j][q][3];
+            RowStager<float, NT>::put(stage, pxq[q], j * 32 + M::ch(lane, q), v[j][q][0], v[j][q][1], v[j][q][2], v[j][q][3]);
+            if (quad_ok(q)) ss = sumsq4(ss, v[j][q][0], v[j][q][1], v[j][q][2], v[j][q][3]);
           }
       }
       if (row_ok) RowStager<float, NT>::template flush<true>(stage, a.out_raw + pix0 * a.Cout + cb, NPX, nvalid, a.Cout, lane);
     }
     if (has_act) {
-      if (!POOL || !(x & 1)) {
+      if (even) {
 #pragma unroll
         for (int j = 0; j < NT; ++j)
 #pragma unroll
           for (int q = 0; q < 4; ++q) {
             float w0 = v[j][q][0], w1 = v[j][q][1], w2 = v[j][q][2], w3 = v[j][q][3];
             if (relu) { w0 = fmaxf(w0, 0.f); w1 = fmaxf(w1, 0.f); w2 = fmaxf(w2, 0.f); w3 = fmaxf(w3, 0.f); }
-            if (Prec<T>::SPLIT && lane_ok && !((GEN || DG) && (a.mask_act || a.add_src)))
+            if (Prec<T>::SPLIT && quad_ok(q) && !((GEN || DG) && (a.mask_act || a.add_src)))
               mx = fmaxf(fmaxf(mx, fmaxf(fabsf(w0), fabsf(w1))), fmaxf(fabsf(w2), fabsf(w3)));
-            RowStager<T, NT>::put(stage, px, j * 32 + q * 8 + g * 4, w0, w1, w2, w3);
+            RowStager<T, NT>::put(stage, pxq[q], j * 32 + M::ch(lane, q), w0, w1, w2, w3);
           }
       }
       const size_t o = pix0 * a.Cout + cb;
@@ -488,13 +535,13 @@
           float am[4];
 #pragma unroll
           for (int e = 0; e < 4; ++e) {
-            const float t0 = acc[i][j][q * 4 + e], u = acc[i + 1][j][q * 4 + e];
+            const float t0 = M::get(acc[i][j], q, e), u = M::get(acc[i + 1][j], q, e);
             const float rown = u > t0 ? 1.f : 0.f;
             const float t = fmaxf(t0, u);
             const float t2 = lane_xor1(t), r2 = lane_xor1(rown);
             am[e] = t2 > t ? 2.f * r2 + 1.f : 2.f * rown;
           }
-          if (!(x & 1)) RowStager<unsigned char, NT>::put(stage, px, j * 32 + q * 8 + g * 4, am[0], am[1], am[2], am[3]);
+          if (!(lane & 1)) RowStager<unsigned char, NT>::put(stage, pxq[q], j * 32 + M::ch(lane, q), am[0], am[1], am[2], am[3]);
         }
       if (row_ok) RowStager<unsigned char, NT>::flush(stage, a.idx_out + pix0 * a.Cout + cb, NPX, nvalid, a.Cout, lane);
     }
@@ -729,8 +776,8 @@
   if (slot & 1) __builtin_amdgcn_s_setprio(1);
 }
 
-template <typename T, int MT, int NT, int WD, int PF, typename Mid>
-__device__ __forceinline__ void stage_mma(f32x16 (&acc)[MT][NT], const char* cur, const FragOff& fo,
+template <typename T, int MT, int NT, int WD, int PF, int SHAPE = SHAPE_32x32x16, typename Mid>
+__device__ __forceinline__ void stage_mma(typename AccMap<SHAPE>::Tile (&acc)[MT][NT], const char* cur, const FragOff& fo,
                                           WeightRing<T, MT, NT, WD, PF>& ring, Mid&& mid) {
   constexpr int RS = WD + 1;
 #pragma unroll
@@ -760,6 +807,11 @@
         for (int c = 0; c < (kg == 0 ? 2 : 1); ++c)
 #pragma unroll
           for (int j = 0; j < NT; ++j) mma16<T>(acc[i][j], ring.wb[tap % RS][c][j], ring.pf[slot]);
+      } else if constexpr (SHAPE == SHAPE_16x16x32) {
+#pragma unroll
+        for (int c = 0; c < 2; ++c)
+#pragma unroll
+          for (int j = 0; j < NT; ++j) mma32<T>(acc[i][j].t[2 * kg + c], ring.wb[tap % RS][c][j], ring.pf[slot]);
       } else {
 #pragma unroll
         for (int j = 0; j < NT; ++j) mma16<T>(acc[i][j], ring.wb[tap % RS][kg][j], ring.pf[slot]);
@@ -770,9 +822,11 @@
   ring.next_stage();
 }
 
-template <typename T, int MT, int NT, int WM, int WN, bool POOL, int WD, bool UNPOOL = false>
+template <typename T, int MT, int NT, int WM, int WN, bool POOL, int WD, bool UNPOOL = false, int SHAPE = SHAPE_32x32x16>
 __global__ __launch_bounds__(256, NT == 1 ? 3 : 2) void conv3x3_kernel(ConvArgs a) {
   static_assert(WM * WN == 4, "4 waves per block");
+  static_assert(SHAPE == SHAPE_32x32x16 || (sizeof(T) == 2 && !UNPOOL), "16x16x32: bf16 / f16 forward kernels only");
+  using M = AccMap<SHAPE>;
   constexpr int EPL = 16 / sizeof(T), KC = SB / sizeof(T);
   constexpr int TH = WM * MT, HPIX = (TH + 2) * HWID;
   constexpr int NPIECE = (HPIX * 4 + 255) / 256;
@@ -955,20 +1009,20 @@
   };
 
   const int ntg0 = (blockIdx.y * WN + wn) * NT;
-  f32x16 acc[MT][NT];
+  typename M::Tile acc[MT][NT];
 #pragma unroll
   for (int j = 0; j < NT; ++j)
 #pragma unroll
     for (int q = 0; q < 4; ++q) {
       float4 b4 = make_float4(0.f, 0.f, 0.f, 0.f);
-      if (sizeof(T) == 2 && a.bias) b4 = *(const float4*)(a.bias + (ntg0 + j) * 32 + q * 8 + (lane >> 5) * 4);
+      if (sizeof(T) == 2 && a.bias) b4 = *(const float4*)(a.bias + (ntg0 + j) * 32 + M::ch(lane, q));
 #pragma unroll
       for (int i = 0; i < MT; ++i) {
-        acc[i][j][q * 4 + 0] = b4.x; acc[i][j][q * 4 + 1] = b4.y; acc[i][j][q * 4 + 2] = b4.z; acc[i][j][q * 4 + 3] = b4.w;
-      }
-    }
-
-  const FragOff fo = frag_offsets(lane, wm * MT);
+        M::set(acc[i][j], q, 0, b4.x); M::set(acc[i][j], q, 1, b4.y); M::set(acc[i][j], q, 2, b4.z); M::set(acc[i][j], q, 3, b4.w);
+      }
+    }
+
+  const FragOff fo = frag_offsets<SHAPE>(lane, wm * MT);
   constexpr int PF = NT == 1 ? (UNPOOL && sizeof(T) == 2 ? 3 : 4) : 3;
   WeightRing<T, MT, NT, WD, PF> ring;
 #pragma unroll
@@ -995,7 +1049,7 @@
   for (int sg = 0; sg < nstage; ++sg) {
     const bool more = sg + 1 < nstage;
     char* nxt = lds + ((sg + 1) & 1) * BUF;
-    stage_mma<T, MT, NT, WD, PF>(acc, lds + (sg & 1) * BUF, fo, ring, [&](int tap) __attribute__((always_inline)) {
+    stage_mma<T, MT, NT, WD, PF, SHAPE>(acc, lds + (sg & 1) * BUF, fo, ring, [&](int tap) __attribute__((always_inline)) {
       if constexpr (DMA) {
         if (tap == HLA_CONV_DMA_TAP && more) dma_stage(sg + 1, (sg + 1) & 1);
       } else {
@@ -1036,17 +1090,17 @@
         return;
       }
     }
-    if (mode == EPI_ACT) conv_epilogue<T, MT, NT, POOL, EPI_ACT, false, LDSB / 4>(acc, a, b, y0 + wm * MT, x0, ntg0 * 32, red, stager, dsc, addb);
+    if (mode == EPI_ACT) conv_epilogue<T, MT, NT, POOL, EPI_ACT, false, LDSB / 4, SHAPE>(acc, a, b, y0 + wm * MT, x0, ntg0 * 32, red, stager, dsc, addb);
     else if (T16 && RAW_SPECIAL && a.raw16 && mode == EPI_ACT_RAW)
-      conv_epilogue<T, MT, NT, POOL, (T16 && RAW_SPECIAL) ? EPI_ACT_RAW : EPI_GENERIC, T16 && RAW_SPECIAL>(acc, a, b, y0 + wm * MT, x0, ntg0 * 32, red, stager, dsc, addb);
+      conv_epilogue<T, MT, NT, POOL, (T16 && RAW_SPECIAL) ? EPI_ACT_RAW : EPI_GENERIC, T16 && RAW_SPECIAL, 0, SHAPE>(acc, a, b, y0 + wm * MT, x0, ntg0 * 32, red, stager, dsc, addb);
     else if (T16 && a.raw16 && mode == EPI_ACT_RAW_NOBIAS)
-      conv_epilogue<T, MT, NT, POOL, T16 ? EPI_ACT_RAW_NOBIAS : EPI_GENERIC, T16>(acc, a, b, y0 + wm * MT, x0, ntg0 * 32, red, stager, dsc, addb);
-    else if (RAW_SPECIAL && mode == EPI_ACT_RAW) conv_epilogue<T, MT, NT, POOL, RAW_SPECIAL ? EPI_ACT_RAW : EPI_GENERIC>(acc, a, b, y0 + wm * MT, x0, ntg0 * 32, red, stager, dsc, addb);
-    else if (mode == EPI_DGRAD)
-      conv_epilogue<T, MT, NT, POOL, EPI_DGRAD>(acc, a, b, y0 + wm * MT, x0, ntg0 * 32, red, stager, dsc, addb);
+      conv_epilogue<T, MT, NT, POOL, T16 ? EPI_ACT_RAW_NOBIAS : EPI_GENERIC, T16, 0, SHAPE>(acc, a, b, y0 + wm * MT, x0, ntg0 * 32, red, stager, dsc, addb);
+    else if (RAW_SPECIAL && mode == EPI_ACT_RAW) conv_epilogue<T, MT, NT, POOL, RAW_SPECIAL ? EPI_ACT_RAW : EPI_GENERIC, false, 0, SHAPE>(acc, a, b, y0 + wm * MT, x0, ntg0 * 32, red, stager, dsc, addb);
+    else if (SHAPE == SHAPE_32x32x16 && mode == EPI_DGRAD)
+      conv_epilogue<T, MT, NT, POOL, SHAPE == SHAPE_32x32x16 ? EPI_DGRAD : EPI_GENERIC, false, 0, SHAPE>(acc, a, b, y0 + wm * MT, x0, ntg0 * 32, red, stager, dsc, addb);
     else if ((RAW_SPECIAL || sizeof(T) == 2) && mode == EPI_ACT_RAW_NOBIAS)
-      conv_epilogue<T, MT, NT, POOL, (RAW_SPECIAL || sizeof(T) == 2) ? EPI_ACT_RAW_NOBIAS : EPI_GENERIC>(acc, a, b, y0 + wm * MT, x0, ntg0 * 32, red, stager, dsc, addb);
-    else conv_epilogue<T, MT, NT, POOL, EPI_GENERIC>(acc, a, b, y0 + wm * MT, x0, ntg0 * 32, red, stager, dsc, addb);
+      conv_epilogue<T, MT, NT, POOL, (RAW_SPECIAL || sizeof(T) == 2) ? EPI_ACT_RAW_NOBIAS : EPI_GENERIC, false, 0, SHAPE>(acc, a, b, y0 + wm * MT, x0, ntg0 * 32, red, stager, dsc, addb);
+    else conv_epilogue<T, MT, NT, POOL, EPI_GENERIC, false, 0, SHAPE>(acc, a, b, y0 + wm * MT, x0, ntg0 * 32, red, stager, dsc, addb);
   }
   HLA_STAMP(5);
 }
@@ -1353,7 +1407,8 @@
 
 template <typename T>
 __device__ __forceinline__ void pack_weights_body(const float* __restrict__ w, T* __restrict__ out, int Cout, int Cin, int first,
-                                                  size_t e0, size_t stride, const float* __restrict__ b0 = nullptr) {
+                                                  size_t e0, size_t stride, const float* __restrict__ b0 = nullptr,
+                                                  int shape = SHAPE_32x32x16) {
   constexpr int EPL = 16 / sizeof(T), KC = SB / sizeof(T), NFRAG = 32 / (2 * EPL);
   const size_t total = first == 1 ? (size_t)(Cout / 32) * NFRAG * 64 * EPL : (size_t)Cout * Cin * 9;
   for (size_t e = e0; e < total; e += stride) {
@@ -1374,7 +1429,9 @@
       const int nsg = Cin / KC;
       const int sg = r % nsg; r /= nsg;
       const int nt = (int)r;
-      const int cout = nt * 32 + (lane & 31), cin = sg * KC + kg * 2 * EPL + (lane >> 5) * EPL + j;
+      const bool s16 = sizeof(T) == 2 && shape == SHAPE_16x16x32;
+      const int cout = s16 ? nt * 32 + kg * 16 + (lane & 15) : nt * 32 + (lane & 31);
+      const int cin = s16 ? sg * KC + (lane >> 4) * EPL + j : sg * KC + kg * 2 * EPL + (lane >> 5) * EPL + j;
       v = first == 2 ? w[((size_t)cin * Cout + cout) * 9 + (8 - tap)] : w[((size_t)cout * Cin + cin) * 9 + tap];
     }
     out[e] = (T)v;
@@ -1387,13 +1444,15 @@
 struct PackTable {
   const float* w[16]; size_t off[16];
   int cout[16], cin[16], first[16];
+  int shape[16];
   const float* b0;
 };
 template <typename T>
 __global__ void pack_weights_multi_kernel(PackTable tb, char* __restrict__ packed) {
   const int l = blockIdx.y;
   pack_weights_body<T>(tb.w[l], (T*)(packed + tb.off[l]), tb.cout[l], tb.cin[l], tb.first[l],
-                       (size_t)blockIdx.x * blockDim.x + threadIdx.x, (size_t)gridDim.x * blockDim.x, tb.first[l] == 1 ? tb.b0 : nullptr);
+                       (size_t)blockIdx.x * blockDim.x + threadIdx.x, (size_t)gridDim.x * blockDim.x, tb.first[l] == 1 ? tb.b0 : nullptr,
+                       tb.shape[l]);
 }
 
 struct SplitPackTable {
@@ -1564,6 +1623,12 @@
 
 
 constexpr int CONV_SMALL_GRID = 320;
+enum { CONV_CLASS_NT2 = 0,
+       CONV_CLASS_NT2_POOL = 1,
+       CONV_CLASS_NT1 = 2 };
+constexpr int kConvClassShape[3] = {SHAPE_16x16x32, SHAPE_16x16x32, SHAPE_32x32x16};
+constexpr int conv_class(int cout, bool pool) { return cout >= 128 ? (pool ? CONV_CLASS_NT2_POOL : CONV_CLASS_NT2) : CONV_CLASS_NT1; }
+template <typename T, bool BWD> constexpr int conv_shape(int cls) { return (sizeof(T) == 2 && !BWD) ? kConvClassShape[cls] : SHAPE_32x32x16; }
 template <typename T, bool BWD = false>
 static bool launch_conv(hipStream_t st, ConvArgs a, bool pool) {
   if (a.unpool_idx && !(BWD && !pool)) {
@@ -1586,30 +1651,32 @@
   const double bytes = (double)P * ((a.up1 ? a.C1 / 4.0 : a.C1) + a.C2) * es + (double)Po * a.Cout * ((a.out_act ? es : 0) + (a.out_raw ? 4 : 0));
   hla_prof_begin_dyn(a.Cout >= 128 ? (pool ? K_CONV_NT2_POOL : K_CONV_NT2) : (pool ? K_CONV_NT1_POOL : K_CONV_NT1), flops, bytes, st,
                      a.dyn ? a.dyn + a.dyn_desc : nullptr, a.tiles_x * a.tiles_y);
+  constexpr int S_NT2 = conv_shape<T, BWD>(CONV_CLASS_NT2), S_NT2P = conv_shape<T, BWD>(CONV_CLASS_NT2_POOL),
+                S_NT1 = conv_shape<T, BWD>(CONV_CLASS_NT1);
   if constexpr (!BWD) {
     const int gy = big ? a.Cout / 128 : 1;
     if (!a.dyn && !a.sumsq && !a.unpool_idx && a.tiles_x * a.tiles_y * a.B * gy < CONV_SMALL_GRID) {
       a.tiles_y = (a.H - a.row_begin + 3) / 4;
       const dim3 g4(a.tiles_x * a.tiles_y * a.B, gy);
       if (big) {
-        if (pool) hipLaunchKernelGGL((conv3x3_kernel<T, 2, 2, 2, 2, true, 1>), g4, dim3(256), 0, st, a);
-        else hipLaunchKernelGGL((conv3x3_kernel<T, 2, 2, 2, 2, false, 1>), g4, dim3(256), 0, st, a);
+        if (pool) hipLaunchKernelGGL((conv3x3_kernel<T, 2, 2, 2, 2, true, 1, false, S_NT2P>), g4, dim3(256), 0, st, a);
+        else hipLaunchKernelGGL((conv3x3_kernel<T, 2, 2, 2, 2, false, 1, false, S_NT2>), g4, dim3(256), 0, st, a);
       } else {
-        if (pool) hipLaunchKernelGGL((conv3x3_kernel<T, 2, 1, 2, 2, true, 2>), g4, dim3(256), 0, st, a);
-        else hipLaunchKernelGGL((conv3x3_kernel<T, 2, 1, 2, 2, false, 2>), g4, dim3(256), 0, st, a);
+        if (pool) hipLaunchKernelGGL((conv3x3_kernel<T, 2, 1, 2, 2, true, 2, false, S_NT1>), g4, dim3(256), 0, st, a);
+        else hipLaunchKernelGGL((conv3x3_kernel<T, 2, 1, 2, 2, false, 2, false, S_NT1>), g4, dim3(256), 0, st, a);
       }
       hla_prof_end(st);
       return true;
     }
   }
   if (big) {
-    if (pool) hipLaunchKernelGGL((conv3x3_kernel<T, 4, 2, 2, 2, true, 1>), grid, dim3(256), 0, st, a);
-    else if (BWD && a.unpool_idx) hipLaunchKernelGGL((conv3x3_kernel<T, 4, 2, 2, 2, false, 1, BWD>), grid, dim3(256), 0, st, a);
-    else hipLaunchKernelGGL((conv3x3_kernel<T, 4, 2, 2, 2, false, 1>), grid, dim3(256), 0, st, a);
+    if (pool) hipLaunchKernelGGL((conv3x3_kernel<T, 4, 2, 2, 2, true, 1, false, S_NT2P>), grid, dim3(256), 0, st, a);
+    else if (BWD && a.unpool_idx) hipLaunchKernelGGL((conv3x3_kernel<T, 4, 2, 2, 2, false, 1, BWD, S_NT2>), grid, dim3(256), 0, st, a);
+    else hipLaunchKernelGGL((conv3x3_kernel<T, 4, 2, 2, 2, false, 1, false, S_NT2>), grid, dim3(256), 0, st, a);
   } else {
-    if (pool) hipLaunchKernelGGL((conv3x3_kernel<T, 4, 1, 2, 2, true, 2>), grid, dim3(256), 0, st, a);
-    else if (BWD && a.unpool_idx) hipLaunchKernelGGL((conv3x3_kernel<T, 4, 1, 2, 2, false, 2, BWD>), grid, dim3(256), 0, st, a);
-    else hipLaunchKernelGGL((conv3x3_kernel<T, 4, 1, 2, 2, false, 2>), grid, dim3(256), 0, st, a);
+    if (pool) hipLaunchKernelGGL((conv3x3_kernel<T, 4, 1, 2, 2, true, 2, false, S_NT1>), grid, dim3(256), 0, st, a);
+    else if (BWD && a.unpool_idx) hipLaunchKernelGGL((conv3x3_kernel<T, 4, 1, 2, 2, false, 2, BWD, S_NT1>), grid, dim3(256), 0, st, a);
+    else hipLaunchKernelGGL((conv3x3_kernel<T, 4, 1, 2, 2, false, 2, false, S_NT1>), grid, dim3(256), 0, st, a);
   }
   hla_prof_end(st);
   return true;
diff --git a/highlyaccurate_amd/csrc/vgg.hip b/highlyaccurate_amd/csrc/vgg.hip
--- a/highlyaccurate_amd/csrc/vgg.hip
+++ b/highlyaccurate_amd/csrc/vgg.hip
@@ -15,6 +15,7 @@
       if (l >= kPackedLayers && !prm->w[l]) continue;
       tb.w[n] = prm->w[l]; tb.off[n] = packed_offset(l, dtype); tb.cout[n] = kLayers[l].cout; tb.cin[n] = kLayers[l].cin;
       tb.first[n] = l == 0 ? 1 : 0;
+      tb.shape[n] = l >= 2 ? conv_shape<T, false>(conv_class(kLayers[l].cout, kLayers[l].pool != 0)) : SHAPE_32x32x16;
       ++n;
     }
     hla_prof_begin(K_PACK, 0, (double)packed_offset(kAllLayers, dtype) * (1.0 + 4.0 / sizeof(T)), st);
@@ -93,6 +94,11 @@
   auto conv = [&](int l, const void* s1, int C1, int H_, int W_h, void* act, int relu, bool pool, const void* s2 = nullptr,
                   int C2 = 0, int up1 = 0, void* raw = nullptr, double* ss = nullptr, unsigned char* idx = nullptr,
                   int row_begin = 0, int norm_level = -1) {
+    if (pool != (kLayers[l].pool != 0)) {
+      hla_set_error("vgg_forward: layer %d launched with pool = %d, the layer table says %d", l, (int)pool, kLayers[l].pool);
+      launch_ok = false;
+      return;
+    }
     ConvArgs a{};
     a.raw16 = (raw && (flags & HLA_VGG_FEAT16)) ? 1 : 0;
     a.row_begin = row_begin < 0 ? 0 : row_begin;
diff --git a/highlyaccurate_amd/csrc/vgg_layers.h b/highlyaccurate_amd/csrc/vgg_layers.h
--- a/highlyaccurate_amd/csrc/vgg_layers.h
+++ b/highlyaccurate_amd/csrc/vgg_layers.h
@@ -1,9 +1,9 @@
 #pragma once
 #include "common.h"
 
-struct LayerDef { int cin, cout, has_bias; };
+struct LayerDef { int cin, cout, has_bias, pool; };
 static const LayerDef kLayers[13] = {
-    {3, 64, 1}, {64, 64, 1}, {64, 128, 1}, {128, 128, 1}, {128, 256, 1}, {256, 256, 1}, {256, 256, 1},
+    {3, 64, 1, 0}, {64, 64, 1, 1}, {64, 128, 1, 0}, {128, 128, 1, 1}, {128, 256, 1, 0}, {256, 256, 1, 0}, {256, 256, 1, 1},
     {384, 128, 0}, {128, 128, 0}, {192, 64, 0}, {64, 64, 0},
     {128, 64, 0}, {64, 64, 0}};
 constexpr int kPackedLayers = 11;
```

New measurement: 5066 pairs/s, median of 6. 1.01x the previous value.
